# LiliMeng/network_interpretation_imagenet

Measured on AMD Instinct MI355X. Metric: masked-forward-passes/sec (224x224, resnet101), higher is better.
Workload: dtype f16x3 (split-fp16 MFMA, fp32 accumulate); stem conv in fp32 by superposition over superpixels; 1 GPU; resnet101, 512 masks/image x 128 images per GPU (BASELINE configs[2]; x1 GPUs); images_per_gpu=128, masks_per_image=512, forward_batch=2340, num_cus=256, entry=MaskedForwardEngine.score_packed, stem=table, lib_stamp=53ee82e6fdd921c4570974547a85c605b3493926e4b08dbc956d47bbb7fcb210, lib_stamp_matches_tree=True, product_library=True, parallelism=mask-batch shard x1 + one all_gather of scores

## Files before the change

include/mpx.h:

```cpp
#ifndef MPX_H
#define MPX_H

#include <stddef.h>
#include <stdint.h>

#ifdef __cplusplus
extern "C" {
#endif

#define MPX_IMG 224
#define MPX_IMG_PAD 230
#define MPX_NUM_CLASSES 1000

enum {
    MPX_E_ARG = -1,
    MPX_E_STATE = -2,
    MPX_E_NOMEM = -3,
    MPX_E_INTERNAL = -4
};

#define MPX_ARCH_MNIST_NET 1
#define MPX_ARCH_CIFAR_RESNET 2000
#define MPX_ARCH_VGG 3000
#define MPX_ARCH_VGG_BN 3100
#define MPX_ARCH_ALEXNET 4000
#define MPX_ARCH_DENSENET 5000
#define MPX_ARCH_MOBILENET 6000
#define MPX_ARCH_SQUEEZENET 7000
#define MPX_ARCH_GOOGLENET 8000
#define MPX_ARCH_SHUFFLENET 9000
#define MPX_ARCH_EFFICIENTNET 10000
typedef struct mpx_engine mpx_engine;

typedef struct mpx_conv_desc {
    char name[48];
    char bn_name[48];
    int32_t cin, cout, ksize, stride, pad;
    int32_t hin, hout;
    int32_t relu;
    int32_t residual;
    int32_t k_packed;
    int32_t cout_pad;
} mpx_conv_desc;

int mpx_create(int arch_id, int max_batch, int device, mpx_engine** out);
int mpx_destroy(mpx_engine* h);
const char* mpx_last_error(const mpx_engine* h);
int mpx_max_batch(const mpx_engine* h);
int mpx_num_cus(const mpx_engine* h);
int mpx_geometry(const mpx_engine* h, int* image_size, int* in_channels, int* num_classes, int* logit_pitch);
size_t mpx_workspace_bytes(const mpx_engine* h);

int mpx_num_convs(const mpx_engine* h);
int mpx_conv_info(const mpx_engine* h, int i, mpx_conv_desc* out);
int mpx_conv_out_slice(const mpx_engine* h, int i, int* pitch, int* offset);
int mpx_conv_in_slice(const mpx_engine* h, int i, int* pitch, int* offset, int* bf, int* hp);
int mpx_conv_consumer_act(const mpx_engine* h, int i, int* act);

int mpx_set_conv_weights(mpx_engine* h, int i, const float* w, const float* conv_bias, const float* gamma,
                         const float* beta, const float* mean, const float* var, float eps);
int mpx_weights_complete(const mpx_engine* h);

typedef struct mpx_norm_desc {
    char name[64];
    int32_t channels;
    int32_t hw;
} mpx_norm_desc;
int mpx_num_norms(const mpx_engine* h);
int mpx_norm_info(const mpx_engine* h, int k, mpx_norm_desc* out);
int mpx_load_norm(mpx_engine* h, int k, const float* gamma, const float* beta, const float* mean, const float* var, float eps);
int mpx_norm_params(const mpx_engine* h, int k, const float** scale, const float** shift);

typedef struct mpx_dwconv_desc {
    char name[48];
    char bn_name[48];
    int32_t channels;
    int32_t pitch;
    int32_t stride;
    int32_t hin;
    int32_t clamp_in;
} mpx_dwconv_desc;
int mpx_num_dwconvs(const mpx_engine* h);
int mpx_dwconv_info(const mpx_engine* h, int k, mpx_dwconv_desc* out);
int mpx_load_dwconv(mpx_engine* h, int k, const float* w, const float* gamma, const float* beta, const float* mean, const float* var, float eps);
int mpx_dwconv_params(const mpx_engine* h, int k, const float** w, const float** scale, const float** shift);
int mpx_dwconv_layout(const mpx_engine* h, int k, int* linear, int* bf, int* hp);
int mpx_dwconv_shape(const mpx_engine* h, int k, int* ksize, int* act_in, int* act_out);

typedef struct mpx_se_desc {
    char name[48];
    int32_t channels;
    int32_t pitch;
    int32_t q;
    int32_t hw;
} mpx_se_desc;
int mpx_num_se(const mpx_engine* h);
int mpx_se_info(const mpx_engine* h, int k, mpx_se_desc* out);
int mpx_load_se(mpx_engine* h, int k, const float* w1, const float* b1, const float* w2, const float* b2);
int mpx_se_params(const mpx_engine* h, int k, const float** w1, const float** b1, const float** w2, const float** b2);

int mpx_set_conv_tile(mpx_engine* h, int i, int tile);
int mpx_get_conv_tile(const mpx_engine* h, int i);
int mpx_last_conv_kernels(const mpx_engine* h);

int mpx_pack_conv_weights(const mpx_conv_desc* d, const float* w, const float* conv_bias, const float* gamma,
                          const float* beta, const float* mean, const float* var, float eps,
                          uint16_t* w_hi, uint16_t* w_lo, float* scale, float* shift);
int mpx_mask_apply_normalize(mpx_engine* h, const uint8_t* img_u8_hwc, const float* img_f32_chw,
                             const int32_t* seg, const uint8_t* onoff, int M, int S,
                             const float mean[3], const float std[3], int slot0,
                             float* out_f32_nchw, void* stream);

int mpx_stem_table_build(mpx_engine* h, const uint8_t* img_u8_hwc, const float* img_f32_chw, const int32_t* seg, int S,
                         const float mean[3], const float std[3], void* stream);
int mpx_stem_table_apply(mpx_engine* h, const uint8_t* onoff, int M, int S, int slot0, void* stream);

int mpx_mask_apply_minmax(mpx_engine* h, const float* img_f32_chw, const int32_t* seg, const uint8_t* removed,
                          int M, int S, int slot0, float* out_f32_nchw, void* stream);

int mpx_avgpool2_pad(mpx_engine* h, const void* in_hi, const void* in_lo, void* out_hi, void* out_lo, int B,
                     int hin, int cin_p, int cout_p, void* stream);

int mpx_conv_bn_act(mpx_engine* h, int i, const void* in_hi, const void* in_lo,
                    const void* res_hi, const void* res_lo, void* out_hi, void* out_lo,
                    float* out_f32, int B, void* stream);

int mpx_conv_dual_bn_act(mpx_engine* h, int i, const void* in_hi, const void* in_lo, const void* x_hi,
                         const void* x_lo, void* out_hi, void* out_lo, int B, void* stream);
int mpx_set_fusion(mpx_engine* h, int mask);

int mpx_bottleneck_tail(mpx_engine* h, int i, const void* t1_hi, const void* t1_lo, const void* x_hi, const void* x_lo,
                        void* out_hi, void* out_lo, void* next_hi, void* next_lo, int B, void* stream);
int mpx_num_bottleneck_tails(const mpx_engine* h);
int mpx_bottleneck_tail_info(const mpx_engine* h, int k, int* conv2, int* conv3, int* downsample, int* next_conv1);

int mpx_maxpool3x3s2(mpx_engine* h, const void* in_hi, const void* in_lo, void* out_hi,
                     void* out_lo, int B, int hin, int c, void* stream);

int mpx_maxpool2x2s2(mpx_engine* h, const void* in_hi, const void* in_lo, void* out_hi,
                     void* out_lo, int B, int hin, int c, void* stream);

int mpx_maxpool3x3s2p0(mpx_engine* h, const void* in_hi, const void* in_lo, void* out_hi,
                       void* out_lo, int B, int hin, int c, void* stream);

int mpx_maxpool3x3_clip(mpx_engine* h, const void* in_hi, const void* in_lo, void* out_hi, void* out_lo, int B, int hin, int stride, int pad,
                        int pitch, void* stream);
int mpx_num_clip_pools(const mpx_engine* h);
int mpx_clip_pool_info(const mpx_engine* h, int k, int* hin, int* stride, int* pad, int* pitch);

int mpx_concat_bn_relu(mpx_engine* h, const void* fresh_hi, const void* fresh_lo, int g, int fresh_stride, void* raw_hi, void* raw_lo,
                       int c_total, int c_old, const float* scale, const float* shift, void* out_hi, void* out_lo, int c_norm,
                       long long npix, void* stream);

int mpx_avgpool2x2s2(mpx_engine* h, const void* in_hi, const void* in_lo, void* out_hi, void* out_lo, int B, int hin, int c,
                     void* stream);

int mpx_dwconv3x3_bn_relu6(mpx_engine* h, const void* in_hi, const void* in_lo, const float* w, const float* scale, const float* shift,
                           void* out_hi, void* out_lo, int B, int hin, int pitch, int stride, int clamp_in, void* stream);

int mpx_dwconv3x3_bn(mpx_engine* h, const void* in_hi, const void* in_lo, const float* w, const float* scale, const float* shift,
                     void* out_hi, void* out_lo, int B, int hin, int pitch, int stride, void* stream);

int mpx_dwconv_bn_act(mpx_engine* h, const void* in_hi, const void* in_lo, const float* w, const float* scale, const float* shift,
                      void* out_hi, void* out_lo, int B, int hin, int pitch, int ksize, int stride, int act_in, int act_out, void* stream);

int mpx_se_gate(mpx_engine* h, const void* in_hi, const void* in_lo, const float* w1, const float* b1, const float* w2, const float* b2,
                float* gate, int B, int hw, int pitch, int q, void* stream);

int mpx_se_scale(mpx_engine* h, const void* in_hi, const void* in_lo, const float* gate, void* out_hi, void* out_lo, int B, int hw, int pitch,
                 void* stream);

int mpx_shuffle2_concat(mpx_engine* h, const void* a_hi, const void* a_lo, int a_pitch, const void* b_hi, const void* b_lo, int b_pitch,
                        void* out_hi, void* out_lo, int B, int hw, int bf, int hp, void* stream);
int mpx_num_shuffles(const mpx_engine* h);
int mpx_shuffle_info(const mpx_engine* h, int k, int* hw, int* bf, int* hp, int* a_pitch, int* b_pitch);

int mpx_global_avgpool_clamp6(mpx_engine* h, const void* in_hi, const void* in_lo, void* out_hi, void* out_lo, int B, int hw,
                              int c, void* stream);

int mpx_global_avgpool_silu(mpx_engine* h, const void* in_hi, const void* in_lo, void* out_hi, void* out_lo, int B, int hw, int c,
                            void* stream);

int mpx_global_avgpool_logits(mpx_engine* h, const void* in_hi, const void* in_lo, float* out_f32, int B, int hw, int c, int out_pitch,
                              void* stream);

int mpx_stem_conv_maxpool(mpx_engine* h, void* out_hi, void* out_lo, int B, void* stream);

int mpx_global_avgpool(mpx_engine* h, const void* in_hi, const void* in_lo, void* out_hi,
                       void* out_lo, int B, int hw, int c, void* stream);

int mpx_head_softmax_gather(mpx_engine* h, const float* logits, const int32_t* label,
                            float* score, int32_t* pred, int B, void* stream);

int mpx_forward(mpx_engine* h, const int32_t* label, float* score, int32_t* pred,
                float* logits_out, int B, void* stream);

int mpx_heatmap_accumulate(mpx_engine* h, const int32_t* seg, const uint8_t* onoff, const int32_t* pred,
                           const int32_t* label, int M, int S, float* heat, void* stream);

int mpx_input_planes(const mpx_engine* h, void** hi, void** lo);
int mpx_mark_input_staged(mpx_engine* h, int slot0, int M);
int mpx_stem_planes(const mpx_engine* h, void** hi, void** lo);
int mpx_profile_enable(mpx_engine* h, int on);
int mpx_profile_collect(mpx_engine* h, double ms_by_kind[4], long long launches_by_kind[4],
                        double* per_conv_ms);
int mpx_profile_collect_ex(mpx_engine* h, double ms_by_kind[4], long long launches_by_kind[4], double* per_conv_ms,
                           double* per_norm_ms, double* avgpool2_ms);
int mpx_profile_collect_dw(mpx_engine* h, double ms_by_kind[4], long long launches_by_kind[4], double* per_conv_ms,
                           double* per_norm_ms, double* avgpool2_ms, double* per_dw_ms);
int mpx_profile_collect_pool(mpx_engine* h, double ms_by_kind[4], long long launches_by_kind[4], double* per_conv_ms,
                             double* per_norm_ms, double* avgpool2_ms, double* per_dw_ms, double* per_clip_pool_ms);
int mpx_profile_collect_shuffle(mpx_engine* h, double ms_by_kind[4], long long launches_by_kind[4], double* per_conv_ms,
                                double* per_norm_ms, double* avgpool2_ms, double* per_dw_ms, double* per_clip_pool_ms, double* per_shuffle_ms);
int mpx_profile_collect_se(mpx_engine* h, double ms_by_kind[4], long long launches_by_kind[4], double* per_conv_ms, double* per_norm_ms,
                           double* avgpool2_ms, double* per_dw_ms, double* per_clip_pool_ms, double* per_shuffle_ms, double* per_se_gate_ms,
                           double* per_se_scale_ms);
double mpx_flops_per_forward(const mpx_engine* h);

#ifdef __cplusplus
}
#endif
#endif
```

network_interpretation_imagenet_amd/_lib.py:

```python
import ctypes as C
import os

import torch

_HERE = os.path.dirname(os.path.abspath(__file__))
PRODUCT_LIB_PATH = os.path.join(_HERE, "libmpx.so")
LIB_PATH = os.environ.get("MPX_LIB_PATH") or PRODUCT_LIB_PATH

IMG = 224
IMG_PAD = 230
NUM_CLASSES = 1000


class MpxError(RuntimeError):
    pass


class ConvDesc(C.Structure):
    _fields_ = [("name", C.c_char * 48), ("bn_name", C.c_char * 48),
                ("cin", C.c_int32), ("cout", C.c_int32), ("ksize", C.c_int32),
                ("stride", C.c_int32), ("pad", C.c_int32), ("hin", C.c_int32),
                ("hout", C.c_int32), ("relu", C.c_int32), ("residual", C.c_int32),
                ("k_packed", C.c_int32), ("cout_pad", C.c_int32)]


class NormDesc(C.Structure):
    _fields_ = [("name", C.c_char * 64), ("channels", C.c_int32), ("hw", C.c_int32)]


class DwConvDesc(C.Structure):
    _fields_ = [("name", C.c_char * 48), ("bn_name", C.c_char * 48), ("channels", C.c_int32), ("pitch", C.c_int32),
                ("stride", C.c_int32), ("hin", C.c_int32), ("clamp_in", C.c_int32)]


class SeDesc(C.Structure):
    _fields_ = [("name", C.c_char * 48), ("channels", C.c_int32), ("pitch", C.c_int32), ("q", C.c_int32), ("hw", C.c_int32)]


_vp, _i, _f = C.c_void_p, C.c_int, C.c_float
_fp = C.POINTER(C.c_float)

SIGNATURES = {
    "mpx_create": (_i, [_i, _i, _i, C.POINTER(_vp)]),
    "mpx_destroy": (_i, [_vp]),
    "mpx_last_error": (C.c_char_p, [_vp]),
    "mpx_max_batch": (_i, [_vp]),
    "mpx_num_cus": (_i, [_vp]),
    "mpx_workspace_bytes": (C.c_size_t, [_vp]),
    "mpx_num_convs": (_i, [_vp]),
    "mpx_conv_info": (_i, [_vp, _i, C.POINTER(ConvDesc)]),
    "mpx_set_conv_weights": (_i, [_vp, _i, _vp, _vp, _vp, _vp, _vp, _vp, _f]),
    "mpx_geometry": (_i, [_vp, C.POINTER(_i), C.POINTER(_i), C.POINTER(_i), C.POINTER(_i)]),
    "mpx_mask_apply_minmax": (_i, [_vp, _vp, _vp, _vp, _i, _i, _i, _vp, _vp]),
    "mpx_avgpool2_pad": (_i, [_vp, _vp, _vp, _vp, _vp, _i, _i, _i, _i, _vp]),
    "mpx_weights_complete": (_i, [_vp]),
    "mpx_set_conv_tile": (_i, [_vp, _i, _i]),
    "mpx_get_conv_tile": (_i, [_vp, _i]),
    "mpx_last_conv_kernels": (_i, [_vp]),
    "mpx_pack_conv_weights": (_i, [C.POINTER(ConvDesc), _vp, _vp, _vp, _vp, _vp, _vp, _f, _vp, _vp, _vp, _vp]),
    "mpx_mask_apply_normalize": (_i, [_vp, _vp, _vp, _vp, _vp, _i, _i, _fp, _fp, _i, _vp, _vp]),
    "mpx_stem_table_build": (_i, [_vp, _vp, _vp, _vp, _i, _fp, _fp, _vp]),
    "mpx_stem_table_apply": (_i, [_vp, _vp, _i, _i, _i, _vp]),
    "mpx_conv_bn_act": (_i, [_vp, _i, _vp, _vp, _vp, _vp, _vp, _vp, _vp, _i, _vp]),
    "mpx_conv_dual_bn_act": (_i, [_vp, _i, _vp, _vp, _vp, _vp, _vp, _vp, _i, _vp]),
    "mpx_set_fusion": (_i, [_vp, _i]),
    "mpx_bottleneck_tail": (_i, [_vp, _i, _vp, _vp, _vp, _vp, _vp, _vp, _vp, _vp, _i, _vp]),
    "mpx_num_bottleneck_tails": (_i, [_vp]),
    "mpx_bottleneck_tail_info": (_i, [_vp, _i, C.POINTER(_i), C.POINTER(_i), C.POINTER(_i), C.POINTER(_i)]),
    "mpx_stem_conv_maxpool": (_i, [_vp, _vp, _vp, _i, _vp]),
    "mpx_maxpool3x3s2": (_i, [_vp, _vp, _vp, _vp, _vp, _i, _i, _i, _vp]),
    "mpx_maxpool2x2s2": (_i, [_vp, _vp, _vp, _vp, _vp, _i, _i, _i, _vp]),
    "mpx_maxpool3x3s2p0": (_i, [_vp, _vp, _vp, _vp, _vp, _i, _i, _i, _vp]),
    "mpx_global_avgpool": (_i, [_vp, _vp, _vp, _vp, _vp, _i, _i, _i, _vp]),
    "mpx_head_softmax_gather": (_i, [_vp, _vp, _vp, _vp, _vp, _i, _vp]),
    "mpx_forward": (_i, [_vp, _vp, _vp, _vp, _vp, _i, _vp]),
    "mpx_heatmap_accumulate": (_i, [_vp, _vp, _vp, _vp, _vp, _i, _i, _vp, _vp]),
    "mpx_input_planes": (_i, [_vp, C.POINTER(_vp), C.POINTER(_vp)]),
    "mpx_mark_input_staged": (_i, [_vp, _i, _i]),
    "mpx_stem_planes": (_i, [_vp, C.POINTER(_vp), C.POINTER(_vp)]),
    "mpx_profile_enable": (_i, [_vp, _i]),
    "mpx_profile_collect": (_i, [_vp, C.POINTER(C.c_double), C.POINTER(C.c_longlong), C.POINTER(C.c_double)]),
    "mpx_flops_per_forward": (C.c_double, [_vp]),
    "mpx_num_norms": (_i, [_vp]),
    "mpx_norm_info": (_i, [_vp, _i, C.POINTER(NormDesc)]),
    "mpx_load_norm": (_i, [_vp, _i, _vp, _vp, _vp, _vp, _f]),
    "mpx_norm_params": (_i, [_vp, _i, C.POINTER(_vp), C.POINTER(_vp)]),
    "mpx_concat_bn_relu": (_i, [_vp, _vp, _vp, _i, _i, _vp, _vp, _i, _i, _vp, _vp, _vp, _vp, _i, C.c_longlong, _vp]),
    "mpx_avgpool2x2s2": (_i, [_vp, _vp, _vp, _vp, _vp, _i, _i, _i, _vp]),
    "mpx_profile_collect_ex": (_i, [_vp, C.POINTER(C.c_double), C.POINTER(C.c_longlong), C.POINTER(C.c_double), C.POINTER(C.c_double),
                                    C.POINTER(C.c_double)]),
    "mpx_num_dwconvs": (_i, [_vp]),
    "mpx_dwconv_info": (_i, [_vp, _i, C.POINTER(DwConvDesc)]),
    "mpx_load_dwconv": (_i, [_vp, _i, _vp, _vp, _vp, _vp, _vp, _f]),
    "mpx_dwconv_params": (_i, [_vp, _i, C.POINTER(_vp), C.POINTER(_vp), C.POINTER(_vp)]),
    "mpx_dwconv3x3_bn_relu6": (_i, [_vp, _vp, _vp, _vp, _vp, _vp, _vp, _vp, _i, _i, _i, _i, _i, _vp]),
    "mpx_global_avgpool_clamp6": (_i, [_vp, _vp, _vp, _vp, _vp, _i, _i, _i, _vp]),
    "mpx_profile_collect_dw": (_i, [_vp, C.POINTER(C.c_double), C.POINTER(C.c_longlong), C.POINTER(C.c_double), C.POINTER(C.c_double),
                                    C.POINTER(C.c_double), C.POINTER(C.c_double)]),
    "mpx_conv_out_slice": (_i, [_vp, _i, C.POINTER(C.c_int), C.POINTER(C.c_int)]),
    "mpx_global_avgpool_logits": (_i, [_vp, _vp, _vp, _vp, _i, _i, _i, _i, _vp]),
    "mpx_maxpool3x3_clip": (_i, [_vp, _vp, _vp, _vp, _vp, _i, _i, _i, _i, _i, _vp]),
    "mpx_num_clip_pools": (_i, [_vp]),
    "mpx_clip_pool_info": (_i, [_vp, _i, C.POINTER(C.c_int), C.POINTER(C.c_int), C.POINTER(C.c_int), C.POINTER(C.c_int)]),
    "mpx_profile_collect_pool": (_i, [_vp, C.POINTER(C.c_double), C.POINTER(C.c_longlong), C.POINTER(C.c_double), C.POINTER(C.c_double),
                                      C.POINTER(C.c_double), C.POINTER(C.c_double), C.POINTER(C.c_double)]),
    "mpx_dwconv3x3_bn": (_i, [_vp, _vp, _vp, _vp, _vp, _vp, _vp, _vp, _i, _i, _i, _i, _vp]),
    "mpx_dwconv_layout": (_i, [_vp, _i, C.POINTER(C.c_int), C.POINTER(C.c_int), C.POINTER(C.c_int)]),
    "mpx_shuffle2_concat": (_i, [_vp, _vp, _vp, _i, _vp, _vp, _i, _vp, _vp, _i, _i, _i, _i, _vp]),
    "mpx_num_shuffles": (_i, [_vp]),
    "mpx_shuffle_info": (_i, [_vp, _i, C.POINTER(C.c_int), C.POINTER(C.c_int), C.POINTER(C.c_int), C.POINTER(C.c_int), C.POINTER(C.c_int)]),
    "mpx_conv_in_slice": (_i, [_vp, _i, C.POINTER(C.c_int), C.POINTER(C.c_int), C.POINTER(C.c_int), C.POINTER(C.c_int)]),
    "mpx_profile_collect_shuffle": (_i, [_vp, C.POINTER(C.c_double), C.POINTER(C.c_longlong), C.POINTER(C.c_double), C.POINTER(C.c_double),
                                         C.POINTER(C.c_double), C.POINTER(C.c_double), C.POINTER(C.c_double), C.POINTER(C.c_double)]),
    "mpx_conv_consumer_act": (_i, [_vp, _i, C.POINTER(C.c_int)]),
    "mpx_dwconv_shape": (_i, [_vp, _i, C.POINTER(C.c_int), C.POINTER(C.c_int), C.POINTER(C.c_int)]),
    "mpx_dwconv_bn_act": (_i, [_vp, _vp, _vp, _vp, _vp, _vp, _vp, _vp, _i, _i, _i, _i, _i, _i, _i, _vp]),
    "mpx_num_se": (_i, [_vp]),
    "mpx_se_info": (_i, [_vp, _i, C.POINTER(SeDesc)]),
    "mpx_load_se": (_i, [_vp, _i, _vp, _vp, _vp, _vp]),
    "mpx_se_params": (_i, [_vp, _i, C.POINTER(_vp), C.POINTER(_vp), C.POINTER(_vp), C.POINTER(_vp)]),
    "mpx_se_gate": (_i, [_vp, _vp, _vp, _vp, _vp, _vp, _vp, _vp, _i, _i, _i, _i, _vp]),
    "mpx_se_scale": (_i, [_vp, _vp, _vp, _vp, _vp, _vp, _i, _i, _i, _vp]),
    "mpx_global_avgpool_silu": (_i, [_vp, _vp, _vp, _vp, _vp, _i, _i, _i, _vp]),
    "mpx_profile_collect_se": (_i, [_vp, C.POINTER(C.c_double), C.POINTER(C.c_longlong)] + [C.POINTER(C.c_double)] * 8),
}

_lib = None


def load():
    global _lib
    if _lib is None:
        if not os.path.exists(LIB_PATH):
            raise MpxError("HIP extension %s not built; run `python -c 'import __graft_entry__ as g; g.build()'` "
                           "(hipcc --offload-arch=gfx950). There is no CPU fallback." % LIB_PATH)
        if is_probe_build():
            import sys
            sys.stderr.write("mpx: binding %s (MPX_LIB_PATH / with_lib.py) -- NOT the product library %s; probe builds may be timing-only\n"
                             % (LIB_PATH, PRODUCT_LIB_PATH))
        lib = C.CDLL(LIB_PATH)
        for name, (res, args) in SIGNATURES.items():
            fn = getattr(lib, name)
            fn.restype = res
            fn.argtypes = args
        _lib = lib
    return _lib


def is_probe_build():
    return os.path.realpath(LIB_PATH) != os.path.realpath(PRODUCT_LIB_PATH)


def bound_library():
    import hashlib
    h = hashlib.sha256()
    with open(LIB_PATH, "rb") as fh:
        for chunk in iter(lambda: fh.read(1 << 20), b""):
            h.update(chunk)
    stamp = None
    if os.path.exists(LIB_PATH + ".sha256"):
        with open(LIB_PATH + ".sha256") as fh:
            stamp = fh.read().strip()
    return {"lib_path": LIB_PATH, "lib_sha256": h.hexdigest(), "lib_stamp": stamp, "product_library": not is_probe_build()}


def check(handle, rc, what):
    if rc != 0:
        msg = load().mpx_last_error(handle).decode() if handle else ""
        raise MpxError("%s failed (rc=%d): %s" % (what, rc, msg))
```

network_interpretation_imagenet_amd/csrc/mpx_api.hip:

```cpp
#include "../../include/mpx.h"
#include "mpx_kernels.h"
#include "mpx_conv3p.h"
#include "mpx_conv3pp.h"
#include "mpx_conv256.h"
#include "mpx_conv256p.h"
#include "mpx_convx.h"
#include "mpx_convw.h"
#include "mpx_btail.h"
#include "mpx_stemtab.h"
#include "mpx_dw.h"
#include "mpx_fire.h"
#include "mpx_pool3c.h"
#include "mpx_shuffle.h"
#include "mpx_mbconv.h"

#include <algorithm>
#include <cmath>
#include <cstdarg>
#include <initializer_list>
#include <new>
#include <cstdio>
#include <cstdlib>
#include <cstring>
#include <string>
#include <vector>

using namespace mpx;

namespace {

constexpr int kActBufs = 4;
constexpr int kStemK = 7;
constexpr int kProfilePairs = 4096;
constexpr size_t kActElemsPerImage = 112 * 112 * 64;
constexpr size_t kVggActElemsPerImage = 224 * 224 * 64;
constexpr size_t kAlexActElemsPerImage = 55 * 55 * 64;
constexpr size_t kMobileActElemsPerImage = 112 * 112 * 96;
constexpr size_t kSqueezeActElemsPerImage = 111 * 111 * 64;
constexpr size_t kShuffleActElemsPerImage = 112 * 112 * 32;
constexpr size_t kEffActElemsPerImage = 112 * 112 * 96;
constexpr int kSmallCPad = 32;

enum OpKind { OP_CONV = 0, OP_MAXPOOL = 1, OP_AVGPOOL = 2, OP_HEAD = 3, OP_AVGPAD = 4, OP_BTAIL = 5, OP_MAXPOOL2 = 6, OP_MAXPOOL3P0 = 7,
              OP_CATNORM = 8, OP_AVGPOOL2 = 9, OP_DWCONV = 10, OP_AVGPOOL6 = 11, OP_AVGLOGITS = 12, OP_MAXPOOL3C = 13, OP_SHUFFLE = 14,
              OP_SEGATE = 15, OP_SESCALE = 16, OP_AVGPOOLSILU = 17 };
enum Buf { BUF_INPUT = -1, BUF_POOL = -2, BUF_NONE = -3, BUF_STEM = -4 };

struct ConvLayer {
    mpx_conv_desc d;
    half_t* w_hi = nullptr;
    half_t* w_lo = nullptr;
    float* scale = nullptr;
    float* shift = nullptr;
    bool loaded = false;
    bool is_fc = false;
    bool is_stem = false;
    int consumer_act = 0;
    bool has_bias = false;
    int cin_pad = 0;
    int cout_store = 0;
    int y_pitch = 0;
    int y_offset = 0;
    int x_pitch = 0;
    int x_offset = 0;
    int in_bf = 0;
    int in_hp = 0;
    int tile = 0;
    int tile_default = -1;
    int fuse_partner = -1;
    bool fuse_main = false;
    half_t* fw_hi = nullptr;
    half_t* fw_lo = nullptr;
    float* fscale = nullptr;
    float* fshift = nullptr;
    bool fused_loaded = false;
    std::vector<float> hw, hgamma, hbeta, hmean, hvar;
    float heps = 0.f;
};

struct Op {
    int kind;
    int conv;
    int in, out, res;
    int hin, c;
    int in2;
    int z = BUF_NONE;
    int g = 0, ctot = 0;
};

struct NormLayer {
    mpx_norm_desc d;
    float* scale = nullptr;
    float* shift = nullptr;
    bool loaded = false;
};

struct TailBlock {
    int c1 = -1, c2 = -1, c3 = -1, ds = -1, next1 = -1;
    half_t* w3p_hi = nullptr;
    half_t* w3p_lo = nullptr;
    bool ready = false;
};

struct DwLayer {
    mpx_dwconv_desc d;
    bool linear = false;
    int in_bf = 0, in_hp = 0;
    int ksize = 3;
    bool mb = false;
    int act_in = 0, act_out = 0;
    float* w = nullptr;
    float* scale = nullptr;
    float* shift = nullptr;
    bool loaded = false;
};

struct SeLayer {
    mpx_se_desc d;
    float* w1 = nullptr;
    float* b1 = nullptr;
    float* w2 = nullptr;
    float* b2 = nullptr;
    bool loaded = false;
};

constexpr int kProfSubDw = -100;
constexpr int kProfSubPool3c = -1000000;
constexpr int kProfSubShuffle = -2000000;
constexpr int kProfSubSeGate = -3000000;
constexpr int kProfSubSeScale = -4000000;

struct ShuffleOp {
    int side, bf, hp, a_pitch, b_pitch, b_offset;
};

struct ClipPool {
    int hin, stride, pad, pitch;
};

struct ProfRec {
    hipEvent_t t0, t1;
    int kind;
    int conv;
    int sub;
};

}

struct mpx_engine {
    int arch = 0, max_batch = 0, device = 0;
    int num_cus = 256;
    int img = MPX_IMG, in_ch = 3, ncls = MPX_NUM_CLASSES, logit_pitch = MPX_NUM_CLASSES;
    bool small = false;
    bool vgg = false;
    bool alexnet = false;
    bool densenet = false;
    std::vector<NormLayer> norms;
    bool mobilenet = false;
    std::vector<DwLayer> dws;
    bool squeezenet = false;
    bool googlenet = false;
    std::vector<ClipPool> pools3c;
    bool shufflenet = false;
    std::vector<ShuffleOp> shuffles;
    bool efficientnet = false;
    std::vector<SeLayer> ses;
    float* se_gate = nullptr;
    int se_pitch_max = 0;
    int n_act_bufs = kActBufs;
    size_t act_elems_per_image = 0;
    float* k0_scratch = nullptr;
    bool bottleneck = false;
    int feat = 0;
    std::vector<ConvLayer> convs;
    std::vector<Op> ops;
    std::vector<Op> ops_bt;
    std::vector<TailBlock> tails;
    int ops_bt_x = 0;
    bool fuse_bt = true;
    char* arena = nullptr;
    size_t arena_bytes = 0;
    char* tab_arena = nullptr;
    size_t tab_arena_bytes = 0;
    half_t* in_hi = nullptr;
    half_t* in_lo = nullptr;
    half_t* act_hi[kActBufs] = {};
    half_t* act_lo[kActBufs] = {};
    half_t* pool_hi = nullptr;
    half_t* pool_lo = nullptr;
    float* logits = nullptr;
    float* seg_scratch = nullptr;
    half_t* stem_hi = nullptr;
    half_t* stem_lo = nullptr;
    float* stem_w32 = nullptr;
    float* stem_s32 = nullptr;
    float* stem_t32 = nullptr;
    int* tab_cnt = nullptr;
    int* tab_off = nullptr;
    int* tab_lab = nullptr;
    int* tab_heavy = nullptr;
    float* tab_vec = nullptr;
    unsigned* tab_bits = nullptr;
    size_t tab_sizes[4] = {0, 0, 0, 0};
    int tab_S = -1;
    bool stem_w_loaded = false;
    std::vector<uint8_t> slot_src;
    std::string err;
    bool in_forward = false;
    unsigned last_kernels = 0;
    bool fuse_ds = true;
    bool fuse_pool = true;
    bool prof_on = false;
    std::vector<ProfRec> prof_pool;
    int prof_used = 0;
    hipStream_t prof_stream = nullptr;
#ifdef MPX_DIAG
    unsigned long long* stamps = nullptr;
#endif
};

namespace {

int fail(mpx_engine* h, int code, const char* fmt, ...) {
    if (h) {
        char buf[512];
        va_list ap;
        va_start(ap, fmt);
        vsnprintf(buf, sizeof buf, fmt, ap);
        va_end(ap);
        h->err = buf;
    }
    return code;
}

#define MPX_HIP(h, call)                                                                         \
    do {                                                                                         \
        hipError_t e_ = (call);                                                                  \
        if (e_ != hipSuccess)                                                                    \
            return fail((h), (int)e_, "%s failed: %s (%s:%d)", #call, hipGetErrorString(e_),     \
                        __FILE__, __LINE__);                                                     \
    } while (0)

#define MPX_SET_DEVICE(h)                                   \
    do {                                                    \
        if (!(h)->in_forward) MPX_HIP((h), hipSetDevice((h)->device)); \
    } while (0)

size_t round_up(size_t v, size_t a) { return (v + a - 1) / a * a; }

void set_name(char* dst, const std::string& s) {
    std::snprintf(dst, 48, "%s", s.c_str());
}

int default_tile(const mpx_conv_desc& d);
bool patch_eligible(const mpx_conv_desc& d);

int build_topology_small(mpx_engine* h);
int build_topology_vgg(mpx_engine* h);
int build_topology_alexnet(mpx_engine* h);
int build_topology_densenet(mpx_engine* h);
int build_topology_mobilenet(mpx_engine* h);
int build_topology_squeezenet(mpx_engine* h);
int build_topology_googlenet(mpx_engine* h);
int build_topology_shufflenet(mpx_engine* h);
int build_topology_efficientnet(mpx_engine* h);

int build_topology(mpx_engine* h) {
    if (h->arch == MPX_ARCH_MNIST_NET || (h->arch > MPX_ARCH_CIFAR_RESNET && h->arch < MPX_ARCH_CIFAR_RESNET + 1000))
        return build_topology_small(h);
    if (h->arch > MPX_ARCH_VGG && h->arch < MPX_ARCH_VGG_BN + 100) return build_topology_vgg(h);
    if (h->arch >= MPX_ARCH_ALEXNET && h->arch < MPX_ARCH_ALEXNET + 100) return build_topology_alexnet(h);
    if (h->arch >= MPX_ARCH_DENSENET && h->arch < MPX_ARCH_DENSENET + 1000) return build_topology_densenet(h);
    if (h->arch >= MPX_ARCH_MOBILENET && h->arch < MPX_ARCH_MOBILENET + 1000) return build_topology_mobilenet(h);
    if (h->arch >= MPX_ARCH_SQUEEZENET && h->arch < MPX_ARCH_SQUEEZENET + 1000) return build_topology_squeezenet(h);
    if (h->arch >= MPX_ARCH_GOOGLENET && h->arch < MPX_ARCH_GOOGLENET + 1000) return build_topology_googlenet(h);
    if (h->arch >= MPX_ARCH_SHUFFLENET && h->arch < MPX_ARCH_SHUFFLENET + 1000) return build_topology_shufflenet(h);
    if (h->arch >= MPX_ARCH_EFFICIENTNET && h->arch < MPX_ARCH_EFFICIENTNET + 1000) return build_topology_efficientnet(h);
    h->act_elems_per_image = kActElemsPerImage;
    int depths[4];
    switch (h->arch) {
        case 18: depths[0] = 2; depths[1] = 2; depths[2] = 2; depths[3] = 2; h->bottleneck = false; break;
        case 34: depths[0] = 3; depths[1] = 4; depths[2] = 6; depths[3] = 3; h->bottleneck = false; break;
        case 50: depths[0] = 3; depths[1] = 4; depths[2] = 6; depths[3] = 3; h->bottleneck = true; break;
        case 101: depths[0] = 3; depths[1] = 4; depths[2] = 23; depths[3] = 3; h->bottleneck = true; break;
        case 152: depths[0] = 3; depths[1] = 8; depths[2] = 36; depths[3] = 3; h->bottleneck = true; break;
        default: return MPX_E_ARG;
    }
    const int exp = h->bottleneck ? 4 : 1;
    auto add_conv = [&](const std::string& name, const std::string& bn, int cin, int cout, int k, int stride,
                        int pad, int hin, int relu, int residual) {
        ConvLayer L;
        std::memset(&L.d, 0, sizeof L.d);
        set_name(L.d.name, name);
        set_name(L.d.bn_name, bn);
        L.d.cin = cin; L.d.cout = cout; L.d.ksize = k; L.d.stride = stride; L.d.pad = pad;
        L.d.hin = hin; L.d.hout = (hin + 2 * pad - k) / stride + 1;
        L.d.relu = relu; L.d.residual = residual;
        L.is_stem = (cin == 3);
        L.cin_pad = cin;
        L.cout_store = cout;
        L.d.k_packed = L.is_stem ? kStemK * 32 : k * k * cin;
        L.d.cout_pad = (int)round_up(cout, 128);
        L.tile = default_tile(L.d);
        h->convs.push_back(L);
        return (int)h->convs.size() - 1;
    };
    auto add_op = [&](int kind, int conv, int in, int out, int res, int hin, int c, int in2 = BUF_NONE) {
        Op o{kind, conv, in, out, res, hin, c, in2};
        h->ops.push_back(o);
    };
    auto pick = [&](std::initializer_list<int> busy) {
        for (int b = 0; b < kActBufs; ++b) {
            bool used = false;
            for (int u : busy) used |= (u == b);
            if (!used) return b;
        }
        return -100;
    };

    int c = add_conv("conv1", "bn1", 3, 64, 7, 2, 3, 224, 1, 0);
    add_op(OP_CONV, c, BUF_INPUT, 0, BUF_NONE, 0, 0);
    add_op(OP_MAXPOOL, -1, 0, BUF_STEM, BUF_NONE, 112, 64);
    int X = BUF_STEM, cin = 64, hcur = 56;
    const int widths[4] = {64, 128, 256, 512};
    struct BlockRec { int c1, c2, c3, ds, hin; };
    std::vector<BlockRec> blocks;
    for (int s = 0; s < 4; ++s) {
        const int w = widths[s];
        for (int b = 0; b < depths[s]; ++b) {
            const int stride = (b == 0 && s > 0) ? 2 : 1;
            const std::string p = "layer" + std::to_string(s + 1) + "." + std::to_string(b) + ".";
            const bool ds = (b == 0) && (stride != 1 || cin != w * exp);
            const int hout = hcur / stride;
            if (!h->bottleneck) {
                const int T1 = pick({X});
                c = add_conv(p + "conv1", p + "bn1", cin, w, 3, stride, 1, hcur, 1, 0);
                add_op(OP_CONV, c, X, T1, BUF_NONE, 0, 0);
                int res = X, T2 = -100;
                if (ds) {
                    T2 = pick({X, T1});
                    c = add_conv(p + "downsample.0", p + "downsample.1", cin, w * exp, 1, stride, 0, hcur, 0, 0);
                    add_op(OP_CONV, c, X, T2, BUF_NONE, 0, 0);
                    res = T2;
                }
                const int O = pick({X, T1, T2});
                c = add_conv(p + "conv2", p + "bn2", w, w, 3, 1, 1, hout, 1, 1);
                add_op(OP_CONV, c, T1, O, res, 0, 0);
                X = O;
            } else {
                BlockRec R{-1, -1, -1, -1, hcur};
                const int T1 = pick({X});
                R.c1 = c = add_conv(p + "conv1", p + "bn1", cin, w, 1, 1, 0, hcur, 1, 0);
                add_op(OP_CONV, c, X, T1, BUF_NONE, 0, 0);
                const int T2 = pick({X, T1});
                R.c2 = c = add_conv(p + "conv2", p + "bn2", w, w, 3, stride, 1, hcur, 1, 0);
                add_op(OP_CONV, c, T1, T2, BUF_NONE, 0, 0);
                int res = X, dsc = -1;
                if (ds) {
                    const int T3 = pick({X, T1, T2});
                    R.ds = dsc = add_conv(p + "downsample.0", p + "downsample.1", cin, w * exp, 1, stride, 0, hcur, 0, 0);
                    add_op(OP_CONV, dsc, X, T3, BUF_NONE, 0, 0);
                    res = T3;
                }
                R.c3 = c = add_conv(p + "conv3", p + "bn3", w, w * exp, 1, 1, 0, hout, 1, 1);
                add_op(OP_CONV, c, T2, T1, res, 0, 0, ds ? X : BUF_NONE);
                if (ds) {
                    h->convs[c].fuse_partner = dsc; h->convs[c].fuse_main = true;
                    h->convs[dsc].fuse_partner = c;
                }
                blocks.push_back(R);
                X = T1;
            }
            cin = w * exp;
            hcur = hout;
        }
    }
    {
        auto tail_ok = [&](size_t k) {
            if (k + 1 >= blocks.size()) return false;
            const mpx_conv_desc& d2 = h->convs[blocks[k].c2].d;
            const mpx_conv_desc& d3 = h->convs[blocks[k].c3].d;
            const mpx_conv_desc& n1 = h->convs[blocks[k + 1].c1].d;
            if (!(d2.cin == BT_MID && d2.cout == BT_MID && d2.ksize == 3 && d2.stride == 1 && d2.hin == 56)) return false;
            if (!(d3.cin == BT_MID && d3.cout == BT_OUT)) return false;
            if (blocks[k].ds >= 0) {
                const mpx_conv_desc& dd = h->convs[blocks[k].ds].d;
                if (!(dd.cin == BT_MID && dd.stride == 1 && dd.ksize == 1)) return false;
            }
            return n1.cin == BT_OUT && n1.ksize == 1 && n1.stride == 1 && n1.hin == 56 && (n1.cout == 64 || n1.cout == 128) &&
                   !(blocks[k].ds >= 0 && n1.cout != 64);
        };
        bool any = false;
        for (size_t k = 0; k < blocks.size(); ++k) any |= tail_ok(k);
        if (any) {
            std::vector<Op>& out = h->ops_bt;
            out.push_back(h->ops[0]);
            out.push_back(h->ops[1]);
            int Xb = BUF_STEM, T1c = -100;
            for (size_t k = 0; k < blocks.size(); ++k) {
                const BlockRec& R = blocks[k];
                int T1 = T1c;
#ifdef BT_NO_HEAD
                const bool whole = false;
#else
                const bool whole = tail_ok(k) && R.ds >= 0 && T1 < 0;
#endif
                if (T1 < 0 && !whole) {
                    T1 = pick({Xb});
                    out.push_back(Op{OP_CONV, R.c1, Xb, T1, BUF_NONE, 0, 0, BUF_NONE});
                }
                T1c = -100;
                if (tail_ok(k)) {
                    TailBlock tb;
                    tb.c1 = R.c1; tb.c2 = R.c2; tb.c3 = R.c3; tb.ds = R.ds; tb.next1 = blocks[k + 1].c1;
                    h->tails.push_back(tb);
                    if (whole) T1 = BUF_NONE;
                    const int O = pick({Xb, T1}), Z = pick({Xb, T1, O});
                    Op o{OP_BTAIL, (int)h->tails.size() - 1, T1, O, Xb, 0, 0, BUF_NONE};
                    o.z = Z;
                    out.push_back(o);
                    Xb = O;
                    T1c = Z;
                    continue;
                }
                const int T2 = pick({Xb, T1});
                out.push_back(Op{OP_CONV, R.c2, T1, T2, BUF_NONE, 0, 0, BUF_NONE});
                int res = Xb;
                if (R.ds >= 0) {
                    const int T3 = pick({Xb, T1, T2});
                    out.push_back(Op{OP_CONV, R.ds, Xb, T3, BUF_NONE, 0, 0, BUF_NONE});
                    res = T3;
                }
                out.push_back(Op{OP_CONV, R.c3, T2, T1, res, 0, 0, R.ds >= 0 ? Xb : BUF_NONE});
                Xb = T1;
            }
            h->ops_bt_x = Xb;
        }
    }
    h->feat = cin;
    add_op(OP_AVGPOOL, -1, X, BUF_POOL, BUF_NONE, hcur, cin);
    c = add_conv("fc", "", cin, MPX_NUM_CLASSES, 1, 1, 0, 1, 0, 0);
    h->convs[c].is_fc = true;
    add_op(OP_CONV, c, BUF_POOL, BUF_NONE, BUF_NONE, 0, 0);
    add_op(OP_HEAD, -1, BUF_NONE, BUF_NONE, BUF_NONE, 0, 0);
    if (!h->ops_bt.empty()) {
        h->ops_bt.push_back(Op{OP_AVGPOOL, -1, h->ops_bt_x, BUF_POOL, BUF_NONE, hcur, cin, BUF_NONE});
        h->ops_bt.push_back(h->ops[h->ops.size() - 2]);
        h->ops_bt.push_back(h->ops[h->ops.size() - 1]);
    }
    return 0;
}

int build_topology_small(mpx_engine* h) {
    h->small = true;
    h->ncls = 10;
    h->logit_pitch = 16;
    auto add_conv = [&](const std::string& name, const std::string& bn, int cin, int cout, int k, int stride, int pad,
                        int hin, int relu, int residual, bool bias, bool fc) {
        ConvLayer L;
        std::memset(&L.d, 0, sizeof L.d);
        set_name(L.d.name, name);
        set_name(L.d.bn_name, bn);
        L.d.cin = cin; L.d.cout = cout; L.d.ksize = k; L.d.stride = stride; L.d.pad = pad;
        L.d.hin = hin; L.d.hout = (hin + 2 * pad - k) / stride + 1;
        L.d.relu = relu; L.d.residual = residual;
        L.has_bias = bias;
        L.is_fc = fc;
        L.cin_pad = (int)round_up(cin, kSmallCPad);
        L.cout_store = fc ? h->logit_pitch : (int)round_up(cout, kSmallCPad);
        L.d.k_packed = k * k * L.cin_pad;
        L.d.cout_pad = (int)round_up(cout, 128);
        L.tile = default_tile(L.d);
        h->convs.push_back(L);
        return (int)h->convs.size() - 1;
    };
    auto add_op = [&](int kind, int conv, int in, int out, int res, int hin, int c) {
        Op o{kind, conv, in, out, res, hin, c, BUF_NONE};
        h->ops.push_back(o);
    };
    int feat = 0, hlast = 0, X = 0;
    size_t act = 0;
    auto track = [&](int hout, int c) { act = std::max(act, (size_t)hout * hout * round_up(c, kSmallCPad)); };
    if (h->arch == MPX_ARCH_MNIST_NET) {
        h->img = 28; h->in_ch = 1;
        const int cfg[5][3] = {{1, 32, 1}, {32, 32, 1}, {32, 64, 2}, {64, 64, 1}, {64, 128, 2}};
        int hcur = 28, in = BUF_INPUT;
        for (int i = 0; i < 5; ++i) {
            const std::string n = "conv" + std::to_string(i + 1);
            const int c = add_conv(n + ".0", n + ".1", cfg[i][0], cfg[i][1], 3, cfg[i][2], 1, hcur, 1, 0, true, false);
            const int out = (in == 0) ? 1 : 0;
            add_op(OP_CONV, c, in, out, BUF_NONE, 0, 0);
            in = out;
            hcur = h->convs[c].d.hout;
            track(hcur, cfg[i][1]);
        }
        const int c6 = add_conv("conv6", "", 128, 128, 3, 1, 1, hcur, 0, 0, true, false);
        X = (in == 0) ? 1 : 0;
        add_op(OP_CONV, c6, in, X, BUF_NONE, 0, 0);
        feat = 128; hlast = hcur;
        h->feat = feat;
        add_op(OP_AVGPOOL, -1, X, BUF_POOL, BUF_NONE, hlast, feat);
        const int cf = add_conv("fc1", "", feat, 10, 1, 1, 0, 1, 0, 0, true, true);
        add_op(OP_CONV, cf, BUF_POOL, BUF_NONE, BUF_NONE, 0, 0);
    } else {
        const int depth = h->arch - MPX_ARCH_CIFAR_RESNET;
        if (depth < 8 || (depth - 2) % 6 != 0) return MPX_E_ARG;
        const int n = (depth - 2) / 6;
        h->img = 32; h->in_ch = 3;
        int c = add_conv("conv1", "bn1", 3, 16, 3, 1, 1, 32, 1, 0, false, false);
        add_op(OP_CONV, c, BUF_INPUT, 0, BUF_NONE, 0, 0);
        track(32, 16);
        X = 0;
        int inplanes = 16, hcur = 32;
        const int planes_of[3] = {16, 32, 64};
        for (int sidx = 0; sidx < 3; ++sidx) {
            const int planes = planes_of[sidx];
            for (int b = 0; b < n; ++b) {
                const int stride = (sidx > 0 && b == 0) ? 2 : 1;
                const std::string p = "layer" + std::to_string(sidx + 1) + "." + std::to_string(b) + ".";
                int busy[3] = {X, -1, -1};
                auto pick = [&]() {
                    for (int q = 0; q < kActBufs; ++q)
                        if (q != busy[0] && q != busy[1] && q != busy[2]) return q;
                    return -100;
                };
                const int T1 = pick();
                busy[1] = T1;
                c = add_conv(p + "conv1", p + "bn1", inplanes, planes, 3, stride, 1, hcur, 1, 0, false, false);
                add_op(OP_CONV, c, X, T1, BUF_NONE, 0, 0);
                const int hout = h->convs[c].d.hout;
                int res = X;
                if (stride != 1 || inplanes != planes) {
                    const int T2 = pick();
                    busy[2] = T2;
                    add_op(OP_AVGPAD, -1, X, T2, BUF_NONE, hcur, (int)round_up(inplanes, kSmallCPad) * 65536 + (int)round_up(planes, kSmallCPad));
                    res = T2;
                }
                const int O = pick();
                c = add_conv(p + "conv2", p + "bn2", planes, planes, 3, 1, 1, hout, 1, 1, false, false);
                add_op(OP_CONV, c, T1, O, res, 0, 0);
                X = O;
                inplanes = planes;
                hcur = hout;
                track(hcur, planes);
            }
        }
        feat = 64; hlast = hcur;
        h->feat = feat;
        add_op(OP_AVGPOOL, -1, X, BUF_POOL, BUF_NONE, hlast, feat);
        const int cf = add_conv("fc", "", feat, 10, 1, 1, 0, 1, 0, 0, true, true);
        add_op(OP_CONV, cf, BUF_POOL, BUF_NONE, BUF_NONE, 0, 0);
    }
    add_op(OP_HEAD, -1, BUF_NONE, BUF_NONE, BUF_NONE, 0, 0);
    h->act_elems_per_image = act;
    return 0;
}

int build_topology_vgg(mpx_engine* h) {
    const bool bn = h->arch > MPX_ARCH_VGG_BN;
    const int depth = h->arch - (bn ? MPX_ARCH_VGG_BN : MPX_ARCH_VGG);
    constexpr int M = 0;
    static const int cfg_a[] = {64, M, 128, M, 256, 256, M, 512, 512, M, 512, 512, M};
    static const int cfg_b[] = {64, 64, M, 128, 128, M, 256, 256, M, 512, 512, M, 512, 512, M};
    static const int cfg_d[] = {64, 64, M, 128, 128, M, 256, 256, 256, M, 512, 512, 512, M, 512, 512, 512, M};
    static const int cfg_e[] = {64, 64, M, 128, 128, M, 256, 256, 256, 256, M, 512, 512, 512, 512, M, 512, 512, 512, 512, M};
    const int* cfg = nullptr;
    int n = 0;
    switch (depth) {
        case 11: cfg = cfg_a; n = (int)(sizeof cfg_a / sizeof *cfg_a); break;
        case 13: cfg = cfg_b; n = (int)(sizeof cfg_b / sizeof *cfg_b); break;
        case 16: cfg = cfg_d; n = (int)(sizeof cfg_d / sizeof *cfg_d); break;
        case 19: cfg = cfg_e; n = (int)(sizeof cfg_e / sizeof *cfg_e); break;
        default: return MPX_E_ARG;
    }
    h->vgg = true;
    h->n_act_bufs = 2;
    h->act_elems_per_image = kVggActElemsPerImage;
    auto add_conv = [&](const std::string& name, const std::string& bn_name, int cin, int cout, int k, int pad, int hin, int relu, bool fc) {
        ConvLayer L;
        std::memset(&L.d, 0, sizeof L.d);
        set_name(L.d.name, name);
        set_name(L.d.bn_name, bn_name);
        L.d.cin = cin; L.d.cout = cout; L.d.ksize = k; L.d.stride = 1; L.d.pad = pad;
        L.d.hin = hin; L.d.hout = hin + 2 * pad - k + 1;
        L.d.relu = relu;
        L.has_bias = true;
        L.is_fc = fc;
        L.is_stem = (cin == 3);
        L.cin_pad = cin;
        L.cout_store = cout;
        L.d.k_packed = L.is_stem ? k * 32 : k * k * cin;
        L.d.cout_pad = (int)round_up(cout, 128);
        L.tile = default_tile(L.d);
        h->convs.push_back(L);
        return (int)h->convs.size() - 1;
    };
    auto add_op = [&](int kind, int conv, int in, int out, int hin, int c) {
        h->ops.push_back(Op{kind, conv, in, out, BUF_NONE, hin, c, BUF_NONE});
    };
    int X = BUF_INPUT, cin = 3, hcur = MPX_IMG, idx = 0;
    for (int j = 0; j < n; ++j) {
// ... 701 lines not shown
        return launched(h, id);
    }
    if constexpr (DUAL) {
        if (p.k1) {
            if (((p.k1 >> 5) - Cfg::NSX) < 0 || (((p.k1 >> 5) - Cfg::NSX) & 1))
                return fail(h, MPX_E_INTERNAL, "dual conv: k1/32 - ring depth must be even and >= 0");
            hipLaunchKernelGGL((conv_f16x3_kernel<Cfg, true>), dim3((unsigned)tiles), dim3(Cfg::NT), Cfg::LDS, st, p);
            return launched(h, id);
        }
    }
    hipLaunchKernelGGL((conv_f16x3_kernel<Cfg>), dim3((unsigned)tiles), dim3(Cfg::NT), Cfg::LDS, st, p);
    return launched(h, id);
}

int launch_conv256(mpx_engine* h, int id, const ConvLayer& L, ConvParams& p, hipStream_t st) {
    long long tiles;
    if (int rc = conv_tiles(h, p, L.d.cout_pad, Conv256::TC, Conv256::TP, tiles)) return rc;
    hipLaunchKernelGGL(conv256_f16x3_kernel, dim3((unsigned)tiles), dim3(Conv256::NT), Conv256::LDS, st, p);
    return launched(h, id);
}

int launch_conv256p(mpx_engine* h, int id, const ConvLayer& L, ConvParams& p, hipStream_t st) {
    if (p.r_hi) return launch_tile(h, 9, L, p, st);
    long long tiles;
    if (int rc = conv_tiles(h, p, L.d.cout_pad, Conv256P::TC, Conv256P::TP, tiles)) return rc;
    const long long grid = persistent_grid(h, p, tiles);
    if (grid <= 0 || tiles < h->num_cus) return launch_tile(h, 2, L, p, st);
    hipLaunchKernelGGL(conv256p_f16x3_kernel<false>, dim3((unsigned)grid), dim3(Conv256P::NT), Conv256P::LDS, st, p);
    return launched(h, id);
}

bool conv256p_dual_eligible(const ConvLayer& L, const ConvLayer& D) {
    return !L.is_fc && !L.is_stem && L.cin_pad == L.d.cin && D.cin_pad == D.d.cin && conv256_eligible(L.d) && D.d.ksize == 1 && D.d.pad == 0 &&
           D.d.cin % 64 == 0;
}

int launch_conv256p_dual(mpx_engine* h, const ConvLayer& L, ConvParams& p, hipStream_t st) {
    if (p.k1 <= 0 || p.k1 % 64 != 0 || (p.ktot - p.k1) <= 0 || (p.ktot - p.k1) % 64 != 0 || p.r_hi)
        return fail(h, MPX_E_INTERNAL, "dual 256x256 conv: k1 = %d and k2 = %d must be multiples of 64, without a residual operand", p.k1, p.ktot - p.k1);
    long long tiles;
    if (int rc = conv_tiles(h, p, L.d.cout_pad, Conv256P::TC, Conv256P::TP, tiles)) return rc;
    const long long grid = persistent_grid(h, p, tiles);
    if (grid <= 0 || tiles < h->num_cus) return 0;
    hipLaunchKernelGGL(conv256p_f16x3_kernel<true>, dim3((unsigned)grid), dim3(Conv256P::NT), Conv256P::LDS, st, p);
    if (int rc = launched(h, 13)) return rc;
    return 1;
}

int launch_convx(mpx_engine* h, int id, const ConvLayer& L, ConvParams& p, hipStream_t st) {
    long long tiles;
    if (int rc = conv_tiles(h, p, L.d.cout_pad, ConvX::TC, ConvX::TP, tiles)) return rc;
    const long long grid = persistent_grid(h, p, tiles);
    if (grid <= 0 || tiles < h->num_cus) return launch_tile(h, 7, L, p, st);
    hipLaunchKernelGGL(convx_f16x3_kernel, dim3((unsigned)grid), dim3(ConvX::NT), ConvX::LDS, st, p);
    return launched(h, id);
}

int launch_convw(mpx_engine* h, int id, const ConvLayer& L, ConvParams& p, hipStream_t st) {
    if (p.ktot != ConvW::K) return fail(h, MPX_E_INTERNAL, "convw: K = %d (the kernel holds K = %d in registers)", p.ktot, ConvW::K);
    if (!p.relu || !p.r_hi) return launch_tile(h, 10, L, p, st);
    long long tiles;
    if (int rc = conv_tiles(h, p, L.d.cout_pad, ConvW::TC, ConvW::TP, tiles)) return rc;
    const long long grid = persistent_grid(h, p, tiles);
    if (grid <= 0 || tiles < 2LL * h->num_cus) return launch_tile(h, 7, L, p, st);
    hipLaunchKernelGGL((convw_f16x3_kernel<ConvW::K, true>), dim3((unsigned)grid), dim3(ConvW::NT), ConvW::LDS, st, p);
    return launched(h, id);
}

template <class PC>
int launch_conv_patch(mpx_engine* h, int id, const ConvLayer& L, ConvParams& p, hipStream_t st) {
    long long tiles;
    if (int rc = conv_tiles(h, p, L.d.cout_pad, PC::TC, PC::TP, tiles)) return rc;
    p.patch_rows = patch_rows_needed(L.d.hin, PC::TP);
    hipLaunchKernelGGL(conv3x3p_f16x3_kernel<PC>, dim3((unsigned)tiles), dim3(PC::NT), PC::lds_bytes(p.patch_rows), st, p);
    return launched(h, id);
}

template <class PC>
int launch_conv_patchp(mpx_engine* h, int id, const ConvLayer& L, ConvParams& p, hipStream_t st) {
    long long tiles;
    if (int rc = conv_tiles(h, p, L.d.cout_pad, PC::TC, PC::TP, tiles)) return rc;
    const long long grid = persistent_grid(h, p, tiles);
    const int H = L.d.hin;
    const long long padded = (long long)(p.M / (H * H) + 2) * (H + 2) * (H + 2);
    if (grid <= 0 || tiles < h->num_cus || p.r_hi || padded >= (1 << 23)) return launch_conv_patch<PC>(h, 6, L, p, st);
    p.patch_rows = patch_rows_needed(H, PC::TP);
    hipLaunchKernelGGL(conv3x3pp_f16x3_kernel<PC>, dim3((unsigned)grid), dim3(PC::NT), PatchPersistent<PC>::lds_bytes(p.patch_rows), st, p);
    return launched(h, id);
}

int launch_patch(mpx_engine* h, int id, const ConvLayer& L, ConvParams& p, hipStream_t st) {
    if (L.d.cout <= 64) return launch_conv_patch<PatchTile1>(h, id, L, p, st);
    return patch_fits<PatchTile0>(L.d) ? launch_conv_patch<PatchTile0>(h, id, L, p, st) : launch_conv_patch<PatchTile2>(h, id, L, p, st);
}

int launch_patchp(mpx_engine* h, int id, const ConvLayer& L, ConvParams& p, hipStream_t st) {
    return patchp_fits<PatchTile0>(L.d) ? launch_conv_patchp<PatchTile0>(h, id, L, p, st) : launch_conv_patchp<PatchTile2>(h, id, L, p, st);
}

struct TileRow {
    int id;
    LaunchFn launch;
    bool (*eligible)(const mpx_conv_desc&);
    const char* refusal;
    int dual;
    bool split;
};

const TileRow kTiles[] = {
    {0, launch_conv_tile<ConvTile0>, nullptr, nullptr, -1, false},
    {1, launch_conv_tile<ConvTile1>, nullptr, nullptr, -1, false},
    {2, launch_conv_tile<ConvTile2, true>, nullptr, nullptr, 2, false},
    {4, launch_conv_tile<ConvTile4>, nullptr, nullptr, -1, false},
    {6, launch_patch, patch_eligible, "the patch kernel needs a 3x3 stride-1 layer whose input patch fits the LDS", -1, false},
    {7, launch_conv_tile<ConvTile7, true>, nullptr, nullptr, 7, false},
    {9, launch_conv256, conv256_eligible, "the 256x256 kernel runs 1x1 stride-1 layers with cout % 256 == 0 and cin % 64 == 0", -1, true},
    {10, launch_convx, convx_eligible,
     "the persistent expanding-1x1 kernel runs 1x1 stride-1 layers with cout % 256 == 0 and cin % 64 == 0, cin >= 128", 7, false},
    {12, launch_patchp, patchp_eligible,
     "the persistent patch kernel needs a 3x3 stride-1 layer with cout >= 128 and no residual operand whose input patch fits the LDS", -1, false},
    {13, launch_conv256p, conv256p_eligible,
     "the persistent 256x256 kernel runs 1x1 stride-1 layers with cout % 256 == 0, cin % 64 == 0 and no residual operand", -1, true},
    {14, launch_convw, convw_eligible,
     "the weights-in-registers expanding-1x1 kernel runs 1x1 stride-1 layers with cout % 256 == 0 and cin = 256", 7, false},
};

struct KernelLds {
    const void* kernel;
    int bytes;
};
const KernelLds kKernelLds[] = {
    {(const void*)conv_f16x3_kernel<ConvTile0>, ConvTile0::LDS},
    {(const void*)conv_f16x3_kernel<ConvTile1>, ConvTile1::LDS},
    {(const void*)conv_f16x3_kernel<ConvTile1, false, true>, ConvTile1::LDS},
    {(const void*)conv_f16x3_kernel<ConvTile2>, ConvTile2::LDS},
    {(const void*)conv_f16x3_kernel<ConvTile7>, ConvTile7::LDS},
    {(const void*)conv_f16x3_kernel<ConvTile2, true>, ConvTile2::LDS},
    {(const void*)conv_f16x3_kernel<ConvTile7, true>, ConvTile7::LDS},
    {(const void*)conv256_f16x3_kernel, Conv256::LDS},
    {(const void*)convx_f16x3_kernel, ConvX::LDS},
    {(const void*)convw_f16x3_kernel<ConvW::K, true>, ConvW::LDS},
    {(const void*)conv256p_f16x3_kernel<false>, Conv256P::LDS},
    {(const void*)conv256p_f16x3_kernel<true>, Conv256P::LDS},
    {(const void*)conv_f16x3_kernel<ConvTile4>, ConvTile4::LDS},
    {(const void*)conv_f16x3_kernel<ConvTile0, false, false, true>, ConvTile0::LDS},
    {(const void*)conv_f16x3_kernel<ConvTile1, false, false, true>, ConvTile1::LDS},
    {(const void*)conv_f16x3_kernel<ConvTile2, false, false, true>, ConvTile2::LDS},
    {(const void*)conv_f16x3_kernel<ConvTile4, false, false, true>, ConvTile4::LDS},
    {(const void*)conv_f16x3_kernel<ConvTile7, false, false, true>, ConvTile7::LDS},
    {(const void*)btail_f16x3_kernel<BtResC64>, BtResC64::LDS},
    {(const void*)btail_f16x3_kernel<BtResC128>, BtResC128::LDS},
    {(const void*)btail_f16x3_kernel<BtDualC64>, BtDualC64::LDS},
    {(const void*)btail_f16x3_kernel<BtHeadC64>, BtHeadC64::LDS},
    {(const void*)conv3x3p_f16x3_kernel<PatchTile0>, kLdsLimit},
    {(const void*)conv3x3p_f16x3_kernel<PatchTile1>, kLdsLimit},
    {(const void*)conv3x3p_f16x3_kernel<PatchTile2>, kLdsLimit},
    {(const void*)conv3x3pp_f16x3_kernel<PatchTile0>, kLdsLimit},
    {(const void*)conv3x3pp_f16x3_kernel<PatchTile2>, kLdsLimit},
};

const TileRow* find_tile(int id) {
    for (const TileRow& r : kTiles)
        if (r.id == id) return &r;
    return nullptr;
}

bool eligible(const TileRow& r, const ConvLayer& L) {
    return !r.eligible || (!L.is_fc && !L.is_stem && L.cin_pad == L.d.cin && !L.y_pitch && !L.x_pitch && r.eligible(L.d));
}

int launch_tile(mpx_engine* h, int id, const ConvLayer& L, ConvParams& p, hipStream_t st) {
    const TileRow* r = find_tile(id);
    if (!r) return fail(h, MPX_E_INTERNAL, "conv: no kernel for tile id %d", id);
    return r->launch(h, id, L, p, st);
}

int default_tile(const mpx_conv_desc& d) {
    if (d.cout <= 64) return d.ksize >= 3 ? 1 : 4;
#ifndef MPX_PROBE_NO_PERSISTENT_PATCH
    if (patchp_eligible(d) && (d.hout >= 14 || (d.hout == 13 && ((d.cout / 128) & (d.cout / 128 - 1)) == 0))) return 12;
#endif
    if (patch_eligible(d)) return 6;
    if (d.ksize == 3) return 0;
    if (d.ksize == 5 && d.cout % 128 != 0 && d.cout % 64 == 0) return 1;
    if (d.ksize == 6) return 2;
#ifndef MPX_PROBE_NO_CONVW
    if (convw_eligible(d) && d.cout > d.cin && d.hout >= 14) return 14;
#endif
    if (convx_eligible(d) && d.cout > d.cin) return 10;
    if (d.stride == 1 && d.cout > d.cin) return 7;
#ifdef MPX_PROBE_NO_PERSISTENT_256
    if (conv256_eligible(d)) return 9;
#endif
    if (conv256_eligible(d)) return conv256p_eligible(d) ? 13 : 9;
    return 2;
}

int conv_params(mpx_engine* h, const ConvLayer& L, const half_t* in_hi, const half_t* in_lo, half_t* y_hi, half_t* y_lo, int B, ConvParams& p) {
    std::memset(&p, 0, sizeof p);
    p.w_hi = L.w_hi; p.w_lo = L.w_lo; p.scale = L.scale; p.shift = L.shift;
    p.y_hi = y_hi; p.y_lo = y_lo;
    p.cout = L.cout_store;
    p.relu = L.d.relu;
    p.ktot = L.d.k_packed;
    if (L.is_stem) {
        p.x_hi = h->in_hi; p.x_lo = h->in_lo;
        p.hin = MPX_IMG_PAD; p.win = MPX_IMG_PAD; p.pix_stride = 4;
        p.kh = L.d.ksize; p.kw = 1; p.stride = L.d.stride; p.pad = L.d.pad - (MPX_IMG_PAD - MPX_IMG) / 2; p.k_per_tap = L.d.k_packed / L.d.ksize;
    } else {
        p.x_hi = in_hi ? in_hi + L.x_offset : in_hi; p.x_lo = in_lo ? in_lo + L.x_offset : in_lo;
        p.hin = L.d.hin; p.win = L.d.hin; p.pix_stride = L.x_pitch ? L.x_pitch : L.cin_pad;
        p.kh = L.d.ksize; p.kw = L.d.ksize; p.stride = L.d.stride; p.pad = L.d.pad; p.k_per_tap = L.cin_pad;
    }
    p.ho = L.d.hout; p.wo = L.d.hout;
    const long long M = (long long)B * p.ho * p.wo;
    if (M > 0x7fffffffLL) return fail(h, MPX_E_ARG, "batch too large for 32-bit pixel indices");
    p.M = (int)M;
#ifdef MPX_DIAG
    p.stamps = h->stamps;
#endif
    return 0;
}

int launch_conv(mpx_engine* h, int i, const half_t* in_hi, const half_t* in_lo, const half_t* r_hi,
                const half_t* r_lo, half_t* y_hi, half_t* y_lo, float* y_f32, int B, hipStream_t st) {
    const ConvLayer& L = h->convs[i];
    if (!L.loaded) return fail(h, MPX_E_STATE, "layer %d (%s) has no weights", i, L.d.name);
    ConvParams p;
    if (int rc = conv_params(h, L, in_hi, in_lo, y_hi, y_lo, B, p)) return rc;
    if ((long long)B * p.hin * p.win > 0x7fffffffLL) return fail(h, MPX_E_ARG, "batch too large for 32-bit pixel indices");
    p.r_hi = r_hi; p.r_lo = r_lo; p.y_f32 = y_f32;
    if (L.y_pitch) {
        if (r_hi || r_lo || y_f32) return fail(h, MPX_E_ARG, "conv: %s writes a channel slice; it takes no residual operand and no fp32 output", L.d.name);
        p.y_pitch = L.y_pitch;
        p.y_hi += L.y_offset; p.y_lo += L.y_offset;
    }
    ProfScope ps(h, st, OP_CONV, i);
    h->last_kernels = 0;
    const TileRow* row = find_tile(L.tile);
    if (row && row->split && !L.is_stem && !L.y_pitch) {
        const long long M = p.M, tiles_c = (p.cout + Conv256::TC - 1) / Conv256::TC, tiles_p = (M + Conv256::TP - 1) / Conv256::TP;
        const long long total = tiles_p * tiles_c, rounds = total / h->num_cus, rest = total - rounds * h->num_cus;
        const long long howo = (long long)p.ho * p.wo;
        const long long n_a = rounds * h->num_cus / tiles_c * Conv256::TP / howo;
        if (rounds >= 1 && rest > 0 && 2 * rest <= h->num_cus && n_a >= 1 && n_a < B) {
            ConvParams q = p;
            p.M = (int)(n_a * howo);
            int rc = launch_tile(h, L.tile, L, p, st);
            if (rc) return rc;
            const size_t xo = (size_t)n_a * p.hin * p.win * p.pix_stride, yo = (size_t)n_a * howo * p.cout;
            q.M = (int)(M - n_a * howo);
            q.x_hi += xo; q.x_lo += xo;
            q.y_hi += yo; q.y_lo += yo;
            if (q.r_hi) { q.r_hi += yo; q.r_lo += yo; }
            return launch_tile(h, 2, L, q, st);
        }
    }
    return launch_tile(h, L.tile, L, p, st);
}

int launch_conv_fused(mpx_engine* h, int i, const half_t* in_hi, const half_t* in_lo, const half_t* x2_hi,
                      const half_t* x2_lo, half_t* y_hi, half_t* y_lo, int B, hipStream_t st) {
    const ConvLayer& L = h->convs[i];
    if (!L.fuse_main || !L.fused_loaded) return fail(h, MPX_E_STATE, "layer %d (%s) has no fused weights", i, L.d.name);
    const ConvLayer& D = h->convs[L.fuse_partner];
    ConvParams p;
    if (int rc = conv_params(h, L, in_hi, in_lo, y_hi, y_lo, B, p)) return rc;
    if ((long long)B * D.d.hin * D.d.hin > 0x7fffffffLL) return fail(h, MPX_E_ARG, "batch too large for 32-bit pixel indices");
    p.w_hi = L.fw_hi; p.w_lo = L.fw_lo; p.scale = L.fscale; p.shift = L.fshift;
    p.k1 = L.d.cin; p.ktot = L.d.cin + D.d.cin;
    p.x2_hi = x2_hi; p.x2_lo = x2_lo;
    p.hin2 = D.d.hin; p.win2 = D.d.hin; p.pix_stride2 = D.d.cin; p.stride2 = D.d.stride;
    ProfScope ps(h, st, OP_CONV, i);
    h->last_kernels = 0;
    const TileRow* row = find_tile(L.tile);
#ifndef MPX_PROBE_NO_DUAL256P
    if ((L.tile == 9 || L.tile == 10 || L.tile == 13 || L.tile == 14) && conv256p_dual_eligible(L, D)) {
        const int rc = launch_conv256p_dual(h, L, p, st);
        if (rc != 0) return rc < 0 ? rc : 0;
    }
#endif
    return launch_tile(h, row && row->dual >= 0 ? row->dual : 7, L, p, st);
}

bool stem_pool_eligible(const mpx_engine* h) {
    if (h->small || h->googlenet || h->convs.empty()) return false;
    const ConvLayer& L = h->convs[0];
    return L.is_stem && L.d.cout == 64 && L.d.hout == 112 && (L.d.hout / 2) % POOL_PY == 0 && (L.d.hout / 2) % POOL_PX == 0 && L.d.relu;
}

int launch_stem_pool(mpx_engine* h, half_t* y_hi, half_t* y_lo, int B, hipStream_t st) {
    const ConvLayer& L = h->convs[0];
    if (!stem_pool_eligible(h)) return fail(h, MPX_E_STATE, "stem + max pool: this architecture has no 7x7 stem with a max pool");
    if (!L.loaded) return fail(h, MPX_E_STATE, "layer 0 (%s) has no weights", L.d.name);
    ConvParams p;
    if (int rc = conv_params(h, L, nullptr, nullptr, y_hi, y_lo, B, p)) return rc;
    p.n_tiles_c = 1;
    const long long nblocks = (long long)B * (p.ho / 2 / POOL_PY) * (p.wo / 2 / POOL_PX);
    if (nblocks > 0x7fffffffLL) return fail(h, MPX_E_ARG, "conv grid out of range");
    ProfScope ps(h, st, OP_CONV, 0);
    hipLaunchKernelGGL((conv_f16x3_kernel<ConvTile1, false, true>), dim3((unsigned)nblocks), dim3(ConvTile1::NT), ConvTile1::LDS, st, p);
    MPX_HIP(h, hipGetLastError());
    return 0;
}

constexpr int bt_perm_channel(int kpos) {
    const int s = kpos >> 5, q = kpos & 31, g = q >> 3, j = q & 7;
    return 32 * s + (j >> 2) * 16 + 4 * g + (j & 3);
}
constexpr bool bt_perm_is_bijection() {
    bool seen[BT_MID] = {};
    for (int k = 0; k < BT_MID; ++k) {
        const int c = bt_perm_channel(k);
        if (c < 0 || c >= BT_MID || seen[c] || (c >> 5) != (k >> 5)) return false;
        seen[c] = true;
    }
    return true;
}
static_assert(bt_perm_is_bijection(), "K permutation of the block tail's conv3 operand");
static_assert(bt_perm_channel(0) == 0 && bt_perm_channel(3) == 3 && bt_perm_channel(4) == 16 && bt_perm_channel(8) == 4 && bt_perm_channel(36) == 48,
              "K position 8g + j <-> channel (j>>2)*16 + 4g + (j&3): registers 4g..4g+3 of two stacked 16-row accumulator fragments");

int upload_tail_planes(mpx_engine* h, TailBlock& tb, const std::vector<uint16_t>& hi, const std::vector<uint16_t>& lo, int K) {
    std::vector<uint16_t> ph((size_t)BT_OUT * K), pl((size_t)BT_OUT * K);
    for (int row = 0; row < BT_OUT; ++row)
        for (int k = 0; k < K; ++k) {
            const int src = k < BT_MID ? bt_perm_channel(k) : k;
            ph[w_packed_index(row, k, K)] = hi[w_packed_index(row, src, K)];
            pl[w_packed_index(row, k, K)] = lo[w_packed_index(row, src, K)];
        }
    MPX_HIP(h, hipMemcpy(tb.w3p_hi, ph.data(), ph.size() * 2, hipMemcpyHostToDevice));
    MPX_HIP(h, hipMemcpy(tb.w3p_lo, pl.data(), pl.size() * 2, hipMemcpyHostToDevice));
    tb.ready = true;
    return 0;
}

TailBlock* tail_of_conv3(mpx_engine* h, int c3) {
    for (TailBlock& tb : h->tails)
        if (tb.c3 == c3) return &tb;
    return nullptr;
}

bool tails_ready(const mpx_engine* h) {
    if (h->tails.empty()) return false;
    for (const TailBlock& tb : h->tails)
        if (!tb.ready || !h->convs[tb.c2].loaded || !h->convs[tb.next1].loaded || !h->convs[tb.c1].loaded) return false;
    return true;
}

int launch_btail(mpx_engine* h, int ti, const half_t* t_hi, const half_t* t_lo, const half_t* x_hi, const half_t* x_lo,
                 half_t* y_hi, half_t* y_lo, half_t* z_hi, half_t* z_lo, int B, hipStream_t st) {
    const TailBlock& tb = h->tails[ti];
    const ConvLayer& L2 = h->convs[tb.c2];
    const ConvLayer& L3 = h->convs[tb.c3];
    const ConvLayer& N1 = h->convs[tb.next1];
    if (!tb.ready || !L2.loaded || !N1.loaded) return fail(h, MPX_E_STATE, "block tail %s: weights missing", L2.d.name);
    const bool dual = tb.ds >= 0;
    const bool head = t_hi == nullptr;
    if (head && !dual) return fail(h, MPX_E_ARG, "block tail %s: only a block with a downsample branch (64-channel input) can run its own conv1 in the launch", L2.d.name);
    BtParams p;
    std::memset(&p, 0, sizeof p);
    p.t_hi = head ? x_hi : t_hi; p.t_lo = head ? x_lo : t_lo;
    if (head) {
        const ConvLayer& L1 = h->convs[tb.c1];
        if (!L1.loaded) return fail(h, MPX_E_STATE, "block tail %s: weights of %s missing", L2.d.name, L1.d.name);
        if (!(L1.d.cin == BT_MID && L1.d.cout == BT_MID && L1.d.ksize == 1 && L1.d.stride == 1)) return fail(h, MPX_E_INTERNAL, "block tail: %s is not a 64 -> 64 1x1 conv", L1.d.name);
        p.w0_hi = L1.w_hi; p.w0_lo = L1.w_lo; p.sc0 = L1.scale; p.sh0 = L1.shift;
    }
    p.w2_hi = L2.w_hi; p.w2_lo = L2.w_lo; p.sc2 = L2.scale; p.sh2 = L2.shift;
    p.w3_hi = tb.w3p_hi; p.w3_lo = tb.w3p_lo;
    p.sc3 = dual ? L3.fscale : L3.scale; p.sh3 = dual ? L3.fshift : L3.shift;
    p.r_hi = x_hi; p.r_lo = x_lo; p.y_hi = y_hi; p.y_lo = y_lo;
    p.w1_hi = N1.w_hi; p.w1_lo = N1.w_lo; p.sc1 = N1.scale; p.sh1 = N1.shift;
    p.z_hi = z_hi; p.z_lo = z_lo;
    p.B = B; p.H = L2.d.hin; p.W = L2.d.hin;
    if (p.H % BT_TY || p.W % BT_TX) return fail(h, MPX_E_INTERNAL, "block tail: %dx%d map is not a whole number of 8x14 tiles", p.H, p.W);
    p.tiles_x = p.W / BT_TX;
    p.tiles_per_img = (p.H / BT_TY) * p.tiles_x;
    const long long n_tiles = (long long)B * p.tiles_per_img;
    if (n_tiles <= 0 || n_tiles > 0x7fffffffLL) return fail(h, MPX_E_ARG, "block tail: batch out of range");
    p.n_tiles = (int)n_tiles;
#ifdef MPX_DIAG
    p.stamps = h->stamps;
#endif
    const long long resident = 2LL * h->num_cus;
    const unsigned grid = (unsigned)std::min<long long>(resident / 8 * 8, (n_tiles + 7) / 8 * 8);
    ProfScope ps(h, st, OP_CONV, tb.c2);
    if (head) hipLaunchKernelGGL(btail_f16x3_kernel<BtHeadC64>, dim3(grid), dim3(256), BtHeadC64::LDS, st, p);
    else if (dual) hipLaunchKernelGGL(btail_f16x3_kernel<BtDualC64>, dim3(grid), dim3(256), BtDualC64::LDS, st, p);
    else if (N1.d.cout == 128) hipLaunchKernelGGL(btail_f16x3_kernel<BtResC128>, dim3(grid), dim3(256), BtResC128::LDS, st, p);
    else hipLaunchKernelGGL(btail_f16x3_kernel<BtResC64>, dim3(grid), dim3(256), BtResC64::LDS, st, p);
    MPX_HIP(h, hipGetLastError());
    return 0;
}

int build_fused(mpx_engine* h, int main) {
    ConvLayer& L = h->convs[main];
    ConvLayer& D = h->convs[L.fuse_partner];
    const int cout = L.d.cout, k1 = L.d.cin, k2 = D.d.cin, K = k1 + k2, rows = L.d.cout_pad;
    std::vector<uint16_t> hi((size_t)rows * K, 0), lo((size_t)rows * K, 0);
    std::vector<float> sc(rows, 0.f), sh(rows, 0.f), row(K);
    for (int co = 0; co < cout; ++co) {
        const double s3 = (double)L.hgamma[co] / std::sqrt((double)L.hvar[co] + (double)L.heps);
        const double sd = (double)D.hgamma[co] / std::sqrt((double)D.hvar[co] + (double)D.heps);
        double s = std::fmax(std::fabs(s3), std::fabs(sd));
        if (!(s > 0.0) || !std::isfinite(s)) s = 1.0;
        const double r3 = s3 / s, rd = sd / s;
        float mx = 0.f;
        for (int k = 0; k < k1; ++k) { row[k] = (float)((double)L.hw[(size_t)co * k1 + k] * r3); mx = std::fmax(mx, std::fabs(row[k])); }
        for (int k = 0; k < k2; ++k) { row[k1 + k] = (float)((double)D.hw[(size_t)co * k2 + k] * rd); mx = std::fmax(mx, std::fabs(row[k1 + k])); }
        int e = 0;
        if (mx > 0.f && std::isfinite(mx)) {
            int ex;
            std::frexp(mx, &ex);
            e = 10 - ex;
        }
        for (int k = 0; k < K; ++k) {
            const float sv = std::ldexp(row[k], e);
            const half_t vh = (half_t)sv;
            const half_t vl = (half_t)(sv - (float)vh);
            hi[w_packed_index(co, k, K)] = half_bits(vh);
            lo[w_packed_index(co, k, K)] = half_bits(vl);
        }
        sc[co] = (float)std::ldexp(s, -e);
        sh[co] = (float)(((double)L.hbeta[co] - (double)L.hmean[co] * s3) + ((double)D.hbeta[co] - (double)D.hmean[co] * sd));
    }
    MPX_HIP(h, hipMemcpy(L.fw_hi, hi.data(), hi.size() * 2, hipMemcpyHostToDevice));
    MPX_HIP(h, hipMemcpy(L.fw_lo, lo.data(), lo.size() * 2, hipMemcpyHostToDevice));
    MPX_HIP(h, hipMemcpy(L.fscale, sc.data(), sc.size() * 4, hipMemcpyHostToDevice));
    MPX_HIP(h, hipMemcpy(L.fshift, sh.data(), sh.size() * 4, hipMemcpyHostToDevice));
    L.fused_loaded = true;
    if (TailBlock* tb = tail_of_conv3(h, main)) return upload_tail_planes(h, *tb, hi, lo, K);
    return 0;
}

int launch_catnorm(mpx_engine* h, const CatNormParams& p, int norm, hipStream_t st) {
    ProfScope ps(h, st, 2, -1, norm);
    const unsigned long long units = (unsigned long long)p.npix * (unsigned)((p.c_end - p.c_begin) / 8);
    const unsigned grid = (unsigned)std::min<unsigned long long>((units + 255) / 256, (unsigned long long)h->num_cus * 8);
    hipLaunchKernelGGL(concat_bn_relu_kernel, dim3(grid), dim3(256), 0, st, p);
    MPX_HIP(h, hipGetLastError());
    return 0;
}

int launch_dwconv(mpx_engine* h, const DwParams& p, int dw, hipStream_t st, bool linear = false) {
    ProfScope ps(h, st, 2, -1, dw >= 0 ? kProfSubDw - dw : -1);
    if (linear) {
        const int W = p.stride == 1 ? DwRun<1>::W : DwRun<2>::W;
        const unsigned long long units = (unsigned long long)(p.npix / p.ho) * (unsigned)((p.ho + W - 1) / W) * (unsigned)(p.pitch / 8);
        const unsigned grid = (unsigned)std::min<unsigned long long>((units + 255) / 256, (unsigned long long)h->num_cus * (p.stride == 1 ? 8 : 2));
        if (p.stride == 1)
            hipLaunchKernelGGL(dwconv3x3_bn_kernel<1>, dim3(grid), dim3(256), 0, st, p);
        else
            hipLaunchKernelGGL(dwconv3x3_bn_kernel<2>, dim3(grid), dim3(256), 0, st, p);
        MPX_HIP(h, hipGetLastError());
        return 0;
    }
    const unsigned long long units = (unsigned long long)p.npix * (unsigned)(p.pitch / 8);
    const unsigned grid = (unsigned)std::min<unsigned long long>((units + 255) / 256, (unsigned long long)h->num_cus * 8);
    hipLaunchKernelGGL(dwconv3x3_bn_relu6_kernel, dim3(grid), dim3(256), 0, st, p);
    MPX_HIP(h, hipGetLastError());
    return 0;
}

int launch_mbdw(mpx_engine* h, const MbDwParams& p, int ksize, int stride, int dw, hipStream_t st) {
    ProfScope ps(h, st, 2, -1, dw >= 0 ? kProfSubDw - dw : -1);
    const int W = stride == 1 ? 4 : 2;
    const unsigned long long units = (unsigned long long)p.rows * (unsigned)((p.ho + W - 1) / W) * (unsigned)(p.pitch / 8);
    const unsigned grid = (unsigned)std::min<unsigned long long>((units + 255) / 256, (unsigned long long)h->num_cus * (stride == 1 ? 8 : 2));
    if (ksize == 3 && stride == 1) hipLaunchKernelGGL((dwconv_bn_act_kernel<3, 1>), dim3(grid), dim3(256), 0, st, p);
    else if (ksize == 3) hipLaunchKernelGGL((dwconv_bn_act_kernel<3, 2>), dim3(grid), dim3(256), 0, st, p);
    else if (stride == 1) hipLaunchKernelGGL((dwconv_bn_act_kernel<5, 1>), dim3(grid), dim3(256), 0, st, p);
    else hipLaunchKernelGGL((dwconv_bn_act_kernel<5, 2>), dim3(grid), dim3(256), 0, st, p);
    MPX_HIP(h, hipGetLastError());
    return 0;
}

size_t se_gate_lds(int pitch, int q) { return ((size_t)se_gate_slices(pitch) * pitch + pitch + q) * sizeof(float); }

int launch_se_gate(mpx_engine* h, const SeGateParams& p, int B, int k, hipStream_t st) {
    ProfScope ps(h, st, 2, -1, k >= 0 ? kProfSubSeGate - k : -1);
    hipLaunchKernelGGL(se_gate_kernel, dim3((unsigned)B), dim3(256), se_gate_lds(p.pitch, p.q), st, p);
    MPX_HIP(h, hipGetLastError());
    return 0;
}

int launch_se_scale(mpx_engine* h, const SeScaleParams& p, int k, hipStream_t st) {
    ProfScope ps(h, st, 2, -1, k >= 0 ? kProfSubSeScale - k : -1);
    const unsigned grid = (unsigned)std::min<long long>((p.units + 255) / 256, (long long)h->num_cus * 8);
    hipLaunchKernelGGL(se_scale_kernel, dim3(grid), dim3(256), 0, st, p);
    MPX_HIP(h, hipGetLastError());
    return 0;
}

int launch_shuffle(mpx_engine* h, const ShuffleParams& p, int k, hipStream_t st) {
    ProfScope ps(h, st, 2, -1, k >= 0 ? kProfSubShuffle - k : -1);
    const unsigned long long units = (unsigned long long)p.npix * (unsigned)(2 * p.hp / 8);
    const unsigned grid = (unsigned)std::min<unsigned long long>((units + 255) / 256, (unsigned long long)h->num_cus * 8);
    if (p.bf % 8 == 0)
        hipLaunchKernelGGL(shuffle2_concat_kernel<true>, dim3(grid), dim3(256), 0, st, p);
    else
        hipLaunchKernelGGL(shuffle2_concat_kernel<false>, dim3(grid), dim3(256), 0, st, p);
    MPX_HIP(h, hipGetLastError());
    return 0;
}

int launch_pool3c(mpx_engine* h, const half_t* in_hi, const half_t* in_lo, half_t* out_hi, half_t* out_lo, int B, int hin, int stride, int pad,
                  int pitch, int k, hipStream_t st) {
    Pool3cParams p;
    std::memset(&p, 0, sizeof p);
    p.x_hi = in_hi; p.x_lo = in_lo; p.y_hi = out_hi; p.y_lo = out_lo;
    p.hin = hin; p.ho = pool3c_out_side(hin, stride, pad); p.pitch = pitch; p.pad = pad;
    p.runs = (p.ho + (stride == 1 ? Pool3c<1>::W : Pool3c<2>::W) - 1) / (stride == 1 ? Pool3c<1>::W : Pool3c<2>::W);
    p.units = (long long)B * p.ho * p.runs * (pitch / 8);
    ProfScope ps(h, st, 2, -1, k >= 0 ? kProfSubPool3c - k : -1);
    const unsigned grid = (unsigned)std::min<long long>((p.units + 255) / 256, (long long)h->num_cus * 2);
    if (stride == 1)
        hipLaunchKernelGGL(maxpool3x3_clip_kernel<1>, dim3(grid), dim3(256), 0, st, p);
    else
        hipLaunchKernelGGL(maxpool3x3_clip_kernel<2>, dim3(grid), dim3(256), 0, st, p);
    MPX_HIP(h, hipGetLastError());
    return 0;
}

int pack_conv_weights(const mpx_conv_desc* d, int in_bf, int in_hp, const float* w, const float* conv_bias, const float* gamma,
                      const float* beta, const float* mean, const float* var, float eps, uint16_t* w_hi, uint16_t* w_lo, float* scale,
                      float* shift);

}

extern "C" {

int mpx_pack_conv_weights(const mpx_conv_desc* d, const float* w, const float* conv_bias, const float* gamma,
                          const float* beta, const float* mean, const float* var, float eps, uint16_t* w_hi,
                          uint16_t* w_lo, float* scale, float* shift) {
    return pack_conv_weights(d, 0, 0, w, conv_bias, gamma, beta, mean, var, eps, w_hi, w_lo, scale, shift);
}

}

namespace {

int pack_conv_weights(const mpx_conv_desc* d, int in_bf, int in_hp, const float* w, const float* conv_bias, const float* gamma,
                      const float* beta, const float* mean, const float* var, float eps, uint16_t* w_hi, uint16_t* w_lo, float* scale,
                      float* shift) {
    if (!d || !w || !w_hi || !w_lo || !scale || !shift) return MPX_E_ARG;
// ... 845 lines not shown
    hipStream_t st = as_stream(stream);
    ProfScope ps(h, st, 2, -1);
    const int total = B * (c / 8);
    hipLaunchKernelGGL(global_avgpool_silu_kernel, dim3((total + 255) / 256), dim3(256), 0, st, (const half_t*)in_hi, (const half_t*)in_lo,
                       (half_t*)out_hi, (half_t*)out_lo, B, hw, c);
    MPX_HIP(h, hipGetLastError());
    return 0;
}

int mpx_shuffle2_concat(mpx_engine* h, const void* a_hi, const void* a_lo, int a_pitch, const void* b_hi, const void* b_lo, int b_pitch,
                        void* out_hi, void* out_lo, int B, int hw, int bf, int hp, void* stream) {
    if (!h) return MPX_E_ARG;
    auto misaligned = [](const void* q) { return ((uintptr_t)q & 15) != 0; };
    if (!a_hi || !a_lo || !b_hi || !b_lo || !out_hi || !out_lo) return fail(h, MPX_E_ARG, "shuffle2_concat: null pointer");
    if (B <= 0 || hw <= 0 || bf <= 0 || (bf & 1) || hp < bf || (hp & 31) || a_pitch < bf || (a_pitch & 7) || b_pitch < bf || (b_pitch & 7))
        return fail(h, MPX_E_ARG, "shuffle2_concat: B > 0, hw > 0, bf even and > 0, hp >= bf a multiple of 32, pitches >= bf and multiples of 8");
    if (misaligned(a_hi) || misaligned(a_lo) || misaligned(b_hi) || misaligned(b_lo) || misaligned(out_hi) || misaligned(out_lo))
        return fail(h, MPX_E_ARG, "shuffle2_concat: every pointer must be 16-byte aligned");
    ShuffleParams p;
    std::memset(&p, 0, sizeof p);
    p.a_hi = (const half_t*)a_hi; p.a_lo = (const half_t*)a_lo; p.b_hi = (const half_t*)b_hi; p.b_lo = (const half_t*)b_lo;
    p.y_hi = (half_t*)out_hi; p.y_lo = (half_t*)out_lo;
    p.npix = (long long)B * hw * hw;
    p.a_pitch = a_pitch; p.b_pitch = b_pitch; p.bf = bf; p.hp = hp;
    MPX_SET_DEVICE(h);
    return launch_shuffle(h, p, -1, as_stream(stream));
}

int mpx_num_shuffles(const mpx_engine* h) { return h ? (int)h->shuffles.size() : MPX_E_ARG; }

int mpx_shuffle_info(const mpx_engine* h, int k, int* hw, int* bf, int* hp, int* a_pitch, int* b_pitch) {
    if (!h || k < 0 || k >= (int)h->shuffles.size()) return MPX_E_ARG;
    const ShuffleOp& S = h->shuffles[k];
    if (hw) *hw = S.side;
    if (bf) *bf = S.bf;
    if (hp) *hp = S.hp;
    if (a_pitch) *a_pitch = S.a_pitch;
    if (b_pitch) *b_pitch = S.b_pitch;
    return 0;
}

int mpx_conv_in_slice(const mpx_engine* h, int i, int* pitch, int* offset, int* bf, int* hp) {
    if (!h || i < 0 || i >= (int)h->convs.size()) return MPX_E_ARG;
    const ConvLayer& L = h->convs[i];
    if (pitch) *pitch = L.is_stem ? 4 : (L.x_pitch ? L.x_pitch : L.cin_pad);
    if (offset) *offset = L.x_offset;
    if (bf) *bf = L.in_bf;
    if (hp) *hp = L.in_hp;
    return 0;
}

int mpx_global_avgpool_clamp6(mpx_engine* h, const void* in_hi, const void* in_lo, void* out_hi, void* out_lo, int B, int hw,
                              int c, void* stream) {
    if (!h) return MPX_E_ARG;
    if (!in_hi || !in_lo || !out_hi || !out_lo || B <= 0 || hw <= 0 || c <= 0 || (c & 7) || (long long)B * (c / 8) > 0x7fffffffLL)
        return fail(h, MPX_E_ARG, "global_avgpool_clamp6: bad arguments (c multiple of 8)");
    MPX_SET_DEVICE(h);
    hipStream_t st = as_stream(stream);
    ProfScope ps(h, st, 2, -1);
    const int total = B * (c / 8);
    hipLaunchKernelGGL(global_avgpool_clamp6_kernel, dim3((total + 255) / 256), dim3(256), 0, st, (const half_t*)in_hi,
                       (const half_t*)in_lo, (half_t*)out_hi, (half_t*)out_lo, B, hw, c);
    MPX_HIP(h, hipGetLastError());
    return 0;
}

int mpx_global_avgpool_logits(mpx_engine* h, const void* in_hi, const void* in_lo, float* out_f32, int B, int hw, int c, int out_pitch,
                              void* stream) {
    if (!h) return MPX_E_ARG;
    if (!in_hi || !in_lo || !out_f32 || B <= 0 || hw <= 0 || c <= 0 || (c & 7) || out_pitch < c || (long long)B * (c / 8) > 0x7fffffffLL)
        return fail(h, MPX_E_ARG, "global_avgpool_logits: bad arguments (c a multiple of 8, out_pitch >= c)");
    if (((uintptr_t)in_hi | (uintptr_t)in_lo) & 15) return fail(h, MPX_E_ARG, "global_avgpool_logits: the planes must be 16-byte aligned");
    MPX_SET_DEVICE(h);
    hipStream_t st = as_stream(stream);
    ProfScope ps(h, st, 2, -1);
    const int total = B * (c / 8);
    hipLaunchKernelGGL(global_avgpool_logits_kernel, dim3((total + 255) / 256), dim3(256), 0, st, (const half_t*)in_hi,
                       (const half_t*)in_lo, out_f32, B, hw, c, out_pitch);
    MPX_HIP(h, hipGetLastError());
    return 0;
}

int mpx_conv_out_slice(const mpx_engine* h, int i, int* pitch, int* offset) {
    if (!h || !pitch || !offset || i < 0 || i >= (int)h->convs.size()) return MPX_E_ARG;
    const ConvLayer& L = h->convs[i];
    *pitch = L.y_pitch ? L.y_pitch : L.cout_store;
    *offset = L.y_pitch ? L.y_offset : 0;
    return 0;
}

int mpx_avgpool2x2s2(mpx_engine* h, const void* in_hi, const void* in_lo, void* out_hi, void* out_lo, int B, int hin, int c,
                     void* stream) {
    if (!h) return MPX_E_ARG;
    if (!in_hi || !in_lo || !out_hi || !out_lo || B <= 0 || hin <= 0 || (hin & 1) || c <= 0 || (c & 7))
        return fail(h, MPX_E_ARG, "avgpool2x2s2: bad arguments (hin even and > 0, c a positive multiple of 8)");
    if (((uintptr_t)in_hi | (uintptr_t)in_lo | (uintptr_t)out_hi | (uintptr_t)out_lo) & 15)
        return fail(h, MPX_E_ARG, "avgpool2x2s2: the planes must be 16-byte aligned");
    MPX_SET_DEVICE(h);
    hipStream_t st = as_stream(stream);
    ProfScope ps(h, st, 2, -1, -2);
    const size_t total = (size_t)B * (hin / 2) * (hin / 2) * (c / 8);
    const unsigned grid = (unsigned)std::min<size_t>((total + 255) / 256, (size_t)h->num_cus * 8);
    hipLaunchKernelGGL(avgpool2x2s2_kernel, dim3(grid), dim3(256), 0, st, (const half_t*)in_hi, (const half_t*)in_lo,
                       (half_t*)out_hi, (half_t*)out_lo, B, hin, c);
    MPX_HIP(h, hipGetLastError());
    return 0;
}

int mpx_head_softmax_gather(mpx_engine* h, const float* logits, const int32_t* label, float* score, int32_t* pred,
                            int B, void* stream) {
    if (!h) return MPX_E_ARG;
    if (!logits || !label || !score || !pred || B <= 0) return fail(h, MPX_E_ARG, "head_softmax_gather: null pointer or empty batch");
    MPX_SET_DEVICE(h);
    hipStream_t st = as_stream(stream);
    ProfScope ps(h, st, 3, -1);
    hipLaunchKernelGGL(head_softmax_gather_kernel, dim3((B + 3) / 4), dim3(256), 0, st, logits, label, score, pred, B,
                       h->ncls, h->logit_pitch);
    MPX_HIP(h, hipGetLastError());
    return 0;
}

int mpx_forward(mpx_engine* h, const int32_t* label, float* score, int32_t* pred, float* logits_out, int B,
                void* stream) {
    if (!h) return MPX_E_ARG;
    if (!label || !score || !pred || B <= 0) return fail(h, MPX_E_ARG, "forward: null pointer or empty batch");
    if (B > h->max_batch) return fail(h, MPX_E_STATE, "forward: B=%d exceeds max_batch=%d", B, h->max_batch);
    if (mpx_weights_complete(h) != 1) return fail(h, MPX_E_STATE, "forward: weights not loaded for every layer");
    float* logits = logits_out ? logits_out : h->logits;
    MPX_HIP(h, hipSetDevice(h->device));
    struct InForward {
        mpx_engine* e;
        explicit InForward(mpx_engine* e_) : e(e_) { e->in_forward = true; }
        ~InForward() { e->in_forward = false; }
    } scope(h);
    auto hi = [&](int b) -> half_t* { return b == BUF_POOL ? h->pool_hi : (b == BUF_STEM ? h->stem_hi : (b >= 0 ? h->act_hi[b] : nullptr)); };
    auto lo = [&](int b) -> half_t* { return b == BUF_POOL ? h->pool_lo : (b == BUF_STEM ? h->stem_lo : (b >= 0 ? h->act_lo[b] : nullptr)); };
    int rc = 0;
    bool skip_pool = false;
    bool stem_done = false;
    {
        int n_tab = 0, n_k0 = 0;
        for (int i = 0; i < B; ++i) {
            n_tab += h->slot_src[i] == 2;
            n_k0 += h->slot_src[i] == 1;
        }
        if (n_tab && n_tab != B)
            return fail(h, MPX_E_STATE, "forward: %d of the %d slots were staged by mpx_stem_table_apply and %d by mpx_mask_apply_normalize; one forward takes one kind", n_tab, B, n_k0);
        stem_done = n_tab == B;
    }
    bool use_bt = h->fuse_bt && h->fuse_ds && tails_ready(h);
    for (const TailBlock& tb : h->tails)
        for (int li : {tb.c1, tb.c2, tb.c3, tb.next1})
            use_bt = use_bt && h->convs[li].tile == default_tile(h->convs[li].d);
    const std::vector<Op>& ops = use_bt ? h->ops_bt : h->ops;
    for (size_t oi = 0; oi < ops.size(); ++oi) {
        const Op& o = ops[oi];
        if (stem_done && ((o.kind == OP_CONV && o.conv == 0) || (o.kind == OP_MAXPOOL && o.out == BUF_STEM))) continue;
        switch (o.kind) {
            case OP_BTAIL:
                rc = launch_btail(h, o.conv, hi(o.in), lo(o.in), hi(o.res), lo(o.res), hi(o.out), lo(o.out), hi(o.z), lo(o.z), B, as_stream(stream));
                break;
            case OP_CONV:
                if (h->fuse_pool && o.conv == 0 && oi + 1 < ops.size() && ops[oi + 1].kind == OP_MAXPOOL && stem_pool_eligible(h) &&
                    h->convs[0].tile == 1) {
                    const Op& pool = ops[oi + 1];
                    rc = launch_stem_pool(h, hi(pool.out), lo(pool.out), B, as_stream(stream));
                    skip_pool = true;
                    break;
                }
                if (h->fuse_ds && h->convs[o.conv].fuse_partner >= 0) {
                    const ConvLayer& CL = h->convs[o.conv];
                    const ConvLayer& MAIN = CL.fuse_main ? CL : h->convs[CL.fuse_partner];
                    const TileRow* r = find_tile(MAIN.tile);
                    if (MAIN.fused_loaded && r && r->dual >= 0) {
                        if (!CL.fuse_main) break;
                        rc = launch_conv_fused(h, o.conv, hi(o.in), lo(o.in), hi(o.in2), lo(o.in2), hi(o.out), lo(o.out), B, as_stream(stream));
                        break;
                    }
                }
                if (h->convs[o.conv].is_fc)
                    rc = mpx_conv_bn_act(h, o.conv, hi(o.in), lo(o.in), nullptr, nullptr, nullptr, nullptr, logits, B, stream);
                else
                    rc = mpx_conv_bn_act(h, o.conv, hi(o.in), lo(o.in), hi(o.res), lo(o.res), hi(o.out), lo(o.out), nullptr, B, stream);
                break;
            case OP_MAXPOOL:
                if (skip_pool) { skip_pool = false; break; }
                rc = mpx_maxpool3x3s2(h, hi(o.in), lo(o.in), hi(o.out), lo(o.out), B, o.hin, o.c, stream);
                break;
            case OP_MAXPOOL2: rc = mpx_maxpool2x2s2(h, hi(o.in), lo(o.in), hi(o.out), lo(o.out), B, o.hin, o.c, stream); break;
            case OP_MAXPOOL3P0: rc = mpx_maxpool3x3s2p0(h, hi(o.in), lo(o.in), hi(o.out), lo(o.out), B, o.hin, o.c, stream); break;
            case OP_AVGPOOL: rc = mpx_global_avgpool(h, hi(o.in), lo(o.in), hi(o.out), lo(o.out), B, o.hin * o.hin, o.c, stream); break;
            case OP_HEAD: rc = mpx_head_softmax_gather(h, logits, label, score, pred, B, stream); break;
            case OP_AVGPAD: rc = mpx_avgpool2_pad(h, hi(o.in), lo(o.in), hi(o.out), lo(o.out), B, o.hin, o.c >> 16, o.c & 0xffff, stream); break;
            case OP_AVGPOOL2: rc = mpx_avgpool2x2s2(h, hi(o.in), lo(o.in), hi(o.out), lo(o.out), B, o.hin, o.c, stream); break;
            case OP_AVGPOOL6: rc = mpx_global_avgpool_clamp6(h, hi(o.in), lo(o.in), hi(o.out), lo(o.out), B, o.hin * o.hin, o.c, stream); break;
            case OP_AVGLOGITS: rc = mpx_global_avgpool_logits(h, hi(o.in), lo(o.in), logits, B, o.hin * o.hin, o.c, h->logit_pitch, stream); break;
            case OP_MAXPOOL3C: {
                const ClipPool& P = h->pools3c[o.conv];
                rc = launch_pool3c(h, hi(o.in), lo(o.in), hi(o.out), lo(o.out), B, P.hin, P.stride, P.pad, P.pitch, o.conv, as_stream(stream));
                break;
            }
            case OP_DWCONV: {
                const DwLayer& D = h->dws[o.conv];
                if (D.mb) {
                    MbDwParams q;
                    std::memset(&q, 0, sizeof q);
                    q.x_hi = hi(o.in); q.x_lo = lo(o.in); q.y_hi = hi(o.out); q.y_lo = lo(o.out);
                    q.w = D.w; q.scale = D.scale; q.shift = D.shift;
                    q.hin = D.d.hin; q.ho = (D.d.hin - 1) / D.d.stride + 1; q.pitch = D.d.pitch; q.act_in = D.act_in; q.act_out = D.act_out;
                    q.rows = (long long)B * q.ho;
                    rc = launch_mbdw(h, q, D.ksize, D.d.stride, o.conv, as_stream(stream));
                    break;
                }
                DwParams p;
                std::memset(&p, 0, sizeof p);
                p.x_hi = hi(o.in); p.x_lo = lo(o.in); p.y_hi = hi(o.out); p.y_lo = lo(o.out);
                p.w = D.w; p.scale = D.scale; p.shift = D.shift;
                p.hin = D.d.hin; p.ho = (D.d.hin - 1) / D.d.stride + 1; p.pitch = D.d.pitch; p.stride = D.d.stride; p.clamp_in = D.d.clamp_in;
                p.npix = (long long)B * p.ho * p.ho;
                rc = launch_dwconv(h, p, o.conv, as_stream(stream), D.linear);
                break;
            }
            case OP_SEGATE: {
                const SeLayer& E = h->ses[o.conv];
                SeGateParams p;
                std::memset(&p, 0, sizeof p);
                p.x_hi = hi(o.in); p.x_lo = lo(o.in);
                p.w1 = E.w1; p.b1 = E.b1; p.w2 = E.w2; p.b2 = E.b2; p.gate = h->se_gate;
                p.hw = E.d.hw * E.d.hw; p.pitch = E.d.pitch; p.q = E.d.q;
                rc = launch_se_gate(h, p, B, o.conv, as_stream(stream));
                break;
            }
            case OP_SESCALE: {
                const SeLayer& E = h->ses[o.conv];
                SeScaleParams p;
                std::memset(&p, 0, sizeof p);
                p.x_hi = hi(o.in); p.x_lo = lo(o.in); p.gate = h->se_gate; p.y_hi = hi(o.out); p.y_lo = lo(o.out);
                p.pitch = E.d.pitch;
                p.per_image = (long long)E.d.hw * E.d.hw * (E.d.pitch / 8);
                p.units = (long long)B * p.per_image;
                rc = launch_se_scale(h, p, o.conv, as_stream(stream));
                break;
            }
            case OP_AVGPOOLSILU: rc = mpx_global_avgpool_silu(h, hi(o.in), lo(o.in), hi(o.out), lo(o.out), B, o.hin * o.hin, o.c, stream); break;
            case OP_SHUFFLE: {
                const ShuffleOp& S = h->shuffles[o.conv];
                ShuffleParams p;
                std::memset(&p, 0, sizeof p);
                p.a_hi = hi(o.in); p.a_lo = lo(o.in); p.b_hi = hi(o.res) + S.b_offset; p.b_lo = lo(o.res) + S.b_offset;
                p.y_hi = hi(o.out); p.y_lo = lo(o.out);
                p.npix = (long long)B * S.side * S.side;
                p.a_pitch = S.a_pitch; p.b_pitch = S.b_pitch; p.bf = S.bf; p.hp = S.hp;
                rc = launch_shuffle(h, p, o.conv, as_stream(stream));
                break;
            }
            case OP_CATNORM: {
                const NormLayer& nl = h->norms[o.conv];
                CatNormParams p;
                std::memset(&p, 0, sizeof p);
                p.f_hi = hi(o.in); p.f_lo = lo(o.in); p.r_hi = hi(o.res); p.r_lo = lo(o.res); p.y_hi = hi(o.out); p.y_lo = lo(o.out);
                p.scale = nl.scale; p.shift = nl.shift;
                p.npix = (long long)B * o.hin * o.hin;
                p.f_stride = o.g; p.c_total = o.ctot; p.c_old = o.c - o.g; p.c_begin = 0; p.c_end = o.c;
                rc = launch_catnorm(h, p, o.conv, as_stream(stream));
                break;
            }
        }
        if (rc) return rc;
    }
    return 0;
}

int mpx_stem_conv_maxpool(mpx_engine* h, void* out_hi, void* out_lo, int B, void* stream) {
    if (!h) return MPX_E_ARG;
    if (!out_hi || !out_lo || B <= 0) return fail(h, MPX_E_ARG, "stem + max pool: null pointer or empty batch");
    if (B > h->max_batch) return fail(h, MPX_E_STATE, "stem + max pool: B=%d exceeds max_batch=%d", B, h->max_batch);
    MPX_SET_DEVICE(h);
    return launch_stem_pool(h, (half_t*)out_hi, (half_t*)out_lo, B, as_stream(stream));
}

int mpx_set_fusion(mpx_engine* h, int mask) {
    if (!h) return MPX_E_ARG;
    h->fuse_pool = (mask & 1) != 0;
    h->fuse_ds = (mask & 1) != 0;
    h->fuse_bt = (mask & 2) != 0;
    return 0;
}

int mpx_bottleneck_tail(mpx_engine* h, int i, const void* t1_hi, const void* t1_lo, const void* x_hi, const void* x_lo,
                        void* out_hi, void* out_lo, void* next_hi, void* next_lo, int B, void* stream) {
    if (!h) return MPX_E_ARG;
    if (B <= 0 || (t1_hi == nullptr) != (t1_lo == nullptr) || !x_hi || !x_lo || !out_hi || !out_lo || !next_hi || !next_lo)
        return fail(h, MPX_E_ARG, "bottleneck_tail: null planes or empty batch");
    int ti = -1;
    for (size_t k = 0; k < h->tails.size(); ++k)
        if (h->tails[k].c2 == i) ti = (int)k;
    if (ti < 0) return fail(h, MPX_E_ARG, "bottleneck_tail: layer %d is not the conv2 of a block whose tail runs as one launch", i);
    {
        const TailBlock& tb = h->tails[ti];
        const size_t px = (size_t)B * h->convs[tb.c2].d.hin * h->convs[tb.c2].d.hin * sizeof(half_t);
        const size_t c_x = tb.ds >= 0 ? BT_MID : BT_OUT, c_next = (size_t)h->convs[tb.next1].d.cout;
        struct Range { const char* lo; size_t n; const char* what; };
        const Range r[8] = {{(const char*)t1_hi, px * BT_MID, "t1_hi"}, {(const char*)t1_lo, px * BT_MID, "t1_lo"},
                            {(const char*)x_hi, px * c_x, "x_hi"}, {(const char*)x_lo, px * c_x, "x_lo"},
                            {(const char*)out_hi, px * BT_OUT, "out_hi"}, {(const char*)out_lo, px * BT_OUT, "out_lo"},
                            {(const char*)next_hi, px * c_next, "next_hi"}, {(const char*)next_lo, px * c_next, "next_lo"}};
        for (int a = 0; a < 8; ++a)
            for (int b = a + 1; b < 8; ++b)
                if (r[a].lo && r[b].lo && r[a].lo < r[b].lo + r[b].n && r[b].lo < r[a].lo + r[a].n)
                    return fail(h, MPX_E_ARG, "bottleneck_tail: planes %s and %s overlap (all plane pairs must be distinct buffers)", r[a].what, r[b].what);
    }
    MPX_SET_DEVICE(h);
    return launch_btail(h, ti, (const half_t*)t1_hi, (const half_t*)t1_lo, (const half_t*)x_hi, (const half_t*)x_lo, (half_t*)out_hi,
                        (half_t*)out_lo, (half_t*)next_hi, (half_t*)next_lo, B, as_stream(stream));
}

int mpx_num_bottleneck_tails(const mpx_engine* h) { return h ? (int)h->tails.size() : MPX_E_ARG; }

int mpx_bottleneck_tail_info(const mpx_engine* h, int k, int* conv2, int* conv3, int* downsample, int* next_conv1) {
    if (!h || k < 0 || k >= (int)h->tails.size()) return MPX_E_ARG;
    if (conv2) *conv2 = h->tails[k].c2;
    if (conv3) *conv3 = h->tails[k].c3;
    if (downsample) *downsample = h->tails[k].ds;
    if (next_conv1) *next_conv1 = h->tails[k].next1;
    return 0;
}

int mpx_conv_dual_bn_act(mpx_engine* h, int i, const void* in_hi, const void* in_lo, const void* x_hi, const void* x_lo,
                         void* out_hi, void* out_lo, int B, void* stream) {
    if (!h) return MPX_E_ARG;
    if (i < 0 || i >= (int)h->convs.size() || B <= 0) return fail(h, MPX_E_ARG, "conv_dual_bn_act: bad layer index or batch");
    if (!h->convs[i].fuse_main) return fail(h, MPX_E_ARG, "conv_dual_bn_act: layer %d (%s) is not the last conv of a block with a downsample branch", i, h->convs[i].d.name);
    if (!in_hi || !in_lo || !x_hi || !x_lo || !out_hi || !out_lo) return fail(h, MPX_E_ARG, "conv_dual_bn_act: null planes");
    MPX_SET_DEVICE(h);
    return launch_conv_fused(h, i, (const half_t*)in_hi, (const half_t*)in_lo, (const half_t*)x_hi, (const half_t*)x_lo,
                             (half_t*)out_hi, (half_t*)out_lo, B, as_stream(stream));
}

int mpx_heatmap_accumulate(mpx_engine* h, const int32_t* seg, const uint8_t* onoff, const int32_t* pred,
                           const int32_t* label, int M, int S, float* heat, void* stream) {
    if (!h) return MPX_E_ARG;
    if (!seg || !onoff || !pred || !label || !heat || M <= 0 || S <= 0 || S > 4096)
        return fail(h, MPX_E_ARG, "heatmap_accumulate: null pointer, empty M/S or S > 4096");
    MPX_SET_DEVICE(h);
    hipStream_t st = as_stream(stream);
    hipLaunchKernelGGL(heatmap_segment_count_kernel, dim3((S + 255) / 256), dim3(256), 0, st, onoff, pred, label, M, S,
                       h->seg_scratch);
    MPX_HIP(h, hipGetLastError());
    const int npix = h->img * h->img;
    hipLaunchKernelGGL(heatmap_gather_kernel, dim3((npix + 255) / 256), dim3(256), 0, st, seg, h->seg_scratch, S, npix, heat);
    MPX_HIP(h, hipGetLastError());
    return 0;
}

int mpx_input_planes(const mpx_engine* h, void** hi, void** lo) {
    if (!h || !hi || !lo) return MPX_E_ARG;
    *hi = h->in_hi;
    *lo = h->in_lo;
    return 0;
}

int mpx_mark_input_staged(mpx_engine* h, int slot0, int M) {
    if (!h) return MPX_E_ARG;
    if (slot0 < 0 || M <= 0 || (long long)slot0 + M > h->max_batch)
        return fail(h, MPX_E_ARG, "mark_input_staged: slots [%d, %d) outside [0, max_batch=%d)", slot0, slot0 + M, h->max_batch);
    if (h->in_forward) return fail(h, MPX_E_STATE, "mark_input_staged: called during mpx_forward");
    std::fill(h->slot_src.begin() + slot0, h->slot_src.begin() + slot0 + M, (uint8_t)1);
    return 0;
}

int mpx_stem_planes(const mpx_engine* h, void** hi, void** lo) {
    if (!h || !hi || !lo) return MPX_E_ARG;
    *hi = h->stem_hi;
    *lo = h->stem_lo;
    return 0;
}

int mpx_profile_enable(mpx_engine* h, int on) {
    if (!h) return MPX_E_ARG;
    if (on && h->prof_pool.empty()) {
        MPX_SET_DEVICE(h);
        h->prof_pool.resize(kProfilePairs);
        for (ProfRec& r : h->prof_pool) {
            MPX_HIP(h, hipEventCreate(&r.t0));
            MPX_HIP(h, hipEventCreate(&r.t1));
        }
    }
    h->prof_on = on != 0;
    return 0;
}

int mpx_profile_collect(mpx_engine* h, double ms_by_kind[4], long long launches_by_kind[4], double* per_conv_ms) {
    return mpx_profile_collect_ex(h, ms_by_kind, launches_by_kind, per_conv_ms, nullptr, nullptr);
}

int mpx_profile_collect_ex(mpx_engine* h, double ms_by_kind[4], long long launches_by_kind[4], double* per_conv_ms,
                           double* per_norm_ms, double* avgpool2_ms) {
    return mpx_profile_collect_dw(h, ms_by_kind, launches_by_kind, per_conv_ms, per_norm_ms, avgpool2_ms, nullptr);
}

int mpx_profile_collect_dw(mpx_engine* h, double ms_by_kind[4], long long launches_by_kind[4], double* per_conv_ms,
                           double* per_norm_ms, double* avgpool2_ms, double* per_dw_ms) {
    return mpx_profile_collect_pool(h, ms_by_kind, launches_by_kind, per_conv_ms, per_norm_ms, avgpool2_ms, per_dw_ms, nullptr);
}

int mpx_profile_collect_pool(mpx_engine* h, double ms_by_kind[4], long long launches_by_kind[4], double* per_conv_ms,
                             double* per_norm_ms, double* avgpool2_ms, double* per_dw_ms, double* per_clip_pool_ms) {
    return mpx_profile_collect_shuffle(h, ms_by_kind, launches_by_kind, per_conv_ms, per_norm_ms, avgpool2_ms, per_dw_ms, per_clip_pool_ms, nullptr);
}

int mpx_profile_collect_shuffle(mpx_engine* h, double ms_by_kind[4], long long launches_by_kind[4], double* per_conv_ms,
                                double* per_norm_ms, double* avgpool2_ms, double* per_dw_ms, double* per_clip_pool_ms, double* per_shuffle_ms) {
    return mpx_profile_collect_se(h, ms_by_kind, launches_by_kind, per_conv_ms, per_norm_ms, avgpool2_ms, per_dw_ms, per_clip_pool_ms, per_shuffle_ms,
                                  nullptr, nullptr);
}

int mpx_profile_collect_se(mpx_engine* h, double ms_by_kind[4], long long launches_by_kind[4], double* per_conv_ms, double* per_norm_ms,
                           double* avgpool2_ms, double* per_dw_ms, double* per_clip_pool_ms, double* per_shuffle_ms, double* per_se_gate_ms,
                           double* per_se_scale_ms) {
    if (!h || !ms_by_kind || !launches_by_kind) return MPX_E_ARG;
    if (h->prof_used == 0) return 0;
    MPX_SET_DEVICE(h);
    MPX_HIP(h, hipEventSynchronize(h->prof_pool[h->prof_used - 1].t1));
    for (int i = 0; i < h->prof_used; ++i) {
        ProfRec& r = h->prof_pool[i];
        float ms = 0.f;
        MPX_HIP(h, hipEventElapsedTime(&ms, r.t0, r.t1));
        ms_by_kind[r.kind] += ms;
        launches_by_kind[r.kind] += 1;
        if (per_conv_ms && r.kind == OP_CONV && r.conv >= 0) per_conv_ms[r.conv] += ms;
        if (per_norm_ms && r.kind == 2 && r.sub >= 0 && r.sub < (int)h->norms.size()) per_norm_ms[r.sub] += ms;
        if (avgpool2_ms && r.kind == 2 && r.sub == -2) *avgpool2_ms += ms;
        if (per_dw_ms && r.kind == 2 && r.sub <= kProfSubDw && kProfSubDw - r.sub < (int)h->dws.size()) per_dw_ms[kProfSubDw - r.sub] += ms;
        if (per_clip_pool_ms && r.kind == 2 && r.sub <= kProfSubPool3c && kProfSubPool3c - r.sub < (int)h->pools3c.size())
            per_clip_pool_ms[kProfSubPool3c - r.sub] += ms;
        if (per_shuffle_ms && r.kind == 2 && r.sub <= kProfSubShuffle && kProfSubShuffle - r.sub < (int)h->shuffles.size())
            per_shuffle_ms[kProfSubShuffle - r.sub] += ms;
        if (per_se_gate_ms && r.kind == 2 && r.sub <= kProfSubSeGate && kProfSubSeGate - r.sub < (int)h->ses.size())
            per_se_gate_ms[kProfSubSeGate - r.sub] += ms;
        if (per_se_scale_ms && r.kind == 2 && r.sub <= kProfSubSeScale && kProfSubSeScale - r.sub < (int)h->ses.size())
            per_se_scale_ms[kProfSubSeScale - r.sub] += ms;
    }
    h->prof_used = 0;
    return 0;
}

#ifdef MPX_DIAG
int mpx_debug_set_stamps(mpx_engine* h, void* dev_buf) {
    if (!h) return MPX_E_ARG;
    h->stamps = (unsigned long long*)dev_buf;
    return 0;
}
#endif

double mpx_flops_per_forward(const mpx_engine* h) {
    if (!h) return 0.0;
    double macs = 0.0;
    for (const ConvLayer& L : h->convs)
        macs += (double)L.d.hout * L.d.hout * L.d.cout * L.d.cin * L.d.ksize * L.d.ksize;
    for (const DwLayer& D : h->dws) {
        const int ho = (D.d.hin - 1) / D.d.stride + 1;
        macs += (double)ho * ho * D.d.channels * D.ksize * D.ksize;
    }
    for (const SeLayer& E : h->ses) macs += 2.0 * E.d.channels * E.d.q;
    return 2.0 * macs;
}

}
```

network_interpretation_imagenet_amd/csrc/mpx_btail.h:

```cpp
#pragma once
#include "mpx_conv.h"
#include <type_traits>

namespace mpx {

struct BtParams {
    const half_t* t_hi;
    const half_t* t_lo;
    const half_t* w0_hi;
    const half_t* w0_lo;
    const float* sc0;
    const float* sh0;
    const half_t* w2_hi;
    const half_t* w2_lo;
    const float* sc2;
    const float* sh2;
    const half_t* w3_hi;
    const half_t* w3_lo;
    const float* sc3;
    const float* sh3;
    const half_t* r_hi;
    const half_t* r_lo;
    half_t* y_hi;
    half_t* y_lo;
// ... 482 lines not shown
                        const float r = fmaxf(v[j], 0.f);
                        const half_t hi = (half_t)r;
                        t2h[s][b][half * 4 + j] = hi;
                        t2l[s][b][half * 4 + j] = (half_t)__builtin_fmaf((float)hi, -one, r);
                    }
                }
            }

#pragma unroll
        for (int a = 0; a < 4 * H1; ++a)
#pragma unroll
            for (int b = 0; b < 2; ++b) acc1[a][b] = (f4){0.f, 0.f, 0.f, 0.f};

        auto chunk = [&](auto c_tag) {
            constexpr int c = decltype(c_tag)::value;
            constexpr int J0 = JC + c * SC;
            f4 acc3[4][2];
#pragma unroll
            for (int a = 0; a < 4; ++a)
#pragma unroll
                for (int b = 0; b < 2; ++b) acc3[a][b] = (f4){0.f, 0.f, 0.f, 0.f};
            step(std::integral_constant<int, J0>{}, acc3, t2h[0], t2l[0]);
            step(std::integral_constant<int, J0 + 1>{}, acc3, t2h[1], t2l[1]);
            if constexpr (DUAL) {
                step(std::integral_constant<int, J0 + 2>{}, acc3, x0h[0], x0l[0]);
                step(std::integral_constant<int, J0 + 3>{}, acc3, x0h[1], x0l[1]);
            }
            __builtin_amdgcn_sched_barrier(0);
            BT_PHASE(bt_ph[2]);
#pragma unroll
            for (int a = 0; a < 4; ++a) {
                const f4 sc = *(const f4*)(vec + V_SC3 + c * 64 + a * 16 + 4 * lg);
                const f4 sh = *(const f4*)(vec + V_SH3 + c * 64 + a * 16 + 4 * lg);
#pragma unroll
                for (int b = 0; b < 2; ++b) *(f4*)(stg + (b * 16 + lp) * 256 + (((a * 4 + lg) ^ lp) << 4)) = acc3[a][b] * sc + sh;
            }
#pragma unroll
            for (int b = 0; b < 2; ++b) {
                f4 v0[2], v1[2];
#pragma unroll
                for (int k = 0; k < 2; ++k) {
                    const int slot = (2 * b + k) * 8 + (lane >> 3);
                    v0[k] = *(const f4*)(stg + slot * 256 + (((2 * uq) ^ (slot & 15)) << 4));
                    v1[k] = *(const f4*)(stg + slot * 256 + (((2 * uq + 1) ^ (slot & 15)) << 4));
                }
#pragma unroll
                for (int k = 0; k < 2; ++k) {
                    const int u = 2 * b + k;
                    const int slot = u * 8 + (lane >> 3);
                    float v[8] = {v0[k][0], v0[k][1], v0[k][2], v0[k][3], v1[k][0], v1[k][1], v1[k][2], v1[k][3]};
                    if (!DUAL) {
                        const h8 a8 = __builtin_bit_cast(h8, idh[u]);
                        const h8 c8 = __builtin_bit_cast(h8, idl[u]);
#pragma unroll
                        for (int j = 0; j < 8; ++j) v[j] = __builtin_fmaf((float)c8[j], one, __builtin_fmaf((float)a8[j], one, v[j]));
                    }
                    h8 oh, ol;
                    bt_relu_split8(v, one, oh, ol);
                    const int voff = (u_pix[u] * (BT_OUT * 2) + uq * 16) | (u_pix[u] & (int)OOB) | ((BT_ABL & 4) ? (int)OOB : 0);
                    __builtin_amdgcn_raw_buffer_store_b128(__builtin_bit_cast(u4, oh), yh, voff, c * 128, BT_AUX_STORE);
                    __builtin_amdgcn_raw_buffer_store_b128(__builtin_bit_cast(u4, ol), yl, voff, c * 128, BT_AUX_STORE);
                    char* const d = stg + (b * 4 + (uq >> 2) * 2) * 1024 + (slot & 15) * 64 + (((uq & 3) ^ (((slot >> 3) & 1) << 1)) << 4);
                    *(h8*)d = oh;
                    *(h8*)(d + 1024) = ol;
                }
            }
            if (C::late_a(J0 + S3 - 1)) {
#pragma unroll
                for (int i = 0; i < 8; ++i) read_a1((sbase + J0 + S3) & 3, fa[(J0 + S3) & 1], i);
            }
#pragma unroll
            for (int b = 0; b < 2; ++b) {
                cb[0].hi[b] = *(const h8*)(stg + (b * 4 + 0) * 1024 + sb_off);
                cb[0].lo[b] = *(const h8*)(stg + (b * 4 + 1) * 1024 + sb_off);
            }
            __builtin_amdgcn_sched_barrier(0);
            BT_PHASE(bt_ph[3]);
            step(std::integral_constant<int, J0 + S3>{}, &acc1[0], cb[0].hi, cb[0].lo);
            if constexpr (H1 == 1) {
                step(std::integral_constant<int, J0 + S3 + 1>{}, &acc1[0], cb[1].hi, cb[1].lo);
            } else {
                step(std::integral_constant<int, J0 + S3 + 1>{}, &acc1[4], cb[0].hi, cb[0].lo);
                step(std::integral_constant<int, J0 + S3 + 2>{}, &acc1[0], cb[1].hi, cb[1].lo);
                step(std::integral_constant<int, J0 + S3 + 3>{}, &acc1[4], cb[1].hi, cb[1].lo);
            }
            BT_PHASE(bt_ph[4]);
        };
        chunk(std::integral_constant<int, 0>{});
        chunk(std::integral_constant<int, 1>{});
        chunk(std::integral_constant<int, 2>{});
        chunk(std::integral_constant<int, 3>{});

        __builtin_amdgcn_sched_barrier(0);
        h8 zoh[4], zol[4];
#pragma unroll
        for (int hb = 0; hb < H1; ++hb) {
#pragma unroll
            for (int a = 0; a < 4; ++a) {
                const f4 sc = *(const f4*)(vec + V_SC1 + hb * 64 + a * 16 + 4 * lg);
                const f4 sh = *(const f4*)(vec + V_SH1 + hb * 64 + a * 16 + 4 * lg);
#pragma unroll
                for (int b = 0; b < 2; ++b) *(f4*)(stg + (b * 16 + lp) * 256 + (((a * 4 + lg) ^ lp) << 4)) = acc1[hb * 4 + a][b] * sc + sh;
            }
#pragma unroll
            for (int u = 0; u < 4; ++u) {
                const int slot = u * 8 + (lane >> 3);
                const f4 w0 = *(const f4*)(stg + slot * 256 + (((2 * uq) ^ (slot & 15)) << 4));
                const f4 w1 = *(const f4*)(stg + slot * 256 + (((2 * uq + 1) ^ (slot & 15)) << 4));
                const float v[8] = {w0[0], w0[1], w0[2], w0[3], w1[0], w1[1], w1[2], w1[3]};
                bt_relu_split8(v, one, zoh[u], zol[u]);
                if (hb + 1 < H1) {
                    const int voff = (u_pix[u] * (C1 * 2) + uq * 16) | (u_pix[u] & (int)OOB) | ((BT_ABL & 4) ? (int)OOB : 0);
                    __builtin_amdgcn_raw_buffer_store_b128(__builtin_bit_cast(u4, zoh[u]), zh, voff, hb * 128, BT_AUX_STORE);
                    __builtin_amdgcn_raw_buffer_store_b128(__builtin_bit_cast(u4, zol[u]), zl, voff, hb * 128, BT_AUX_STORE);
                }
            }
        }
        __builtin_amdgcn_sched_barrier(0);
        asm volatile("s_waitcnt lgkmcnt(0)" ::: "memory");
        BT_SUB(0);
        __builtin_amdgcn_s_barrier();
        __builtin_amdgcn_sched_barrier(0);
        BT_SUB(2);
        if (it + 1 < my_tiles) issue_patch(it + 1);
        __builtin_amdgcn_sched_barrier(0);
        BT_SUB(4);
#pragma unroll
        for (int u = 0; u < 4; ++u) {
            const int voff = (u_pix[u] * (C1 * 2) + uq * 16) | (u_pix[u] & (int)OOB) | ((BT_ABL & 4) ? (int)OOB : 0);
            __builtin_amdgcn_raw_buffer_store_b128(__builtin_bit_cast(u4, zoh[u]), zh, voff, (H1 - 1) * 128, BT_AUX_STORE);
            __builtin_amdgcn_raw_buffer_store_b128(__builtin_bit_cast(u4, zol[u]), zl, voff, (H1 - 1) * 128, BT_AUX_STORE);
        }
        __builtin_amdgcn_sched_barrier(0);
        BT_SUB(3);
        sbase = (sbase + NSTEP) & 3;
        BT_PHASE(bt_ph[5]);
    }
    wait_vmcnt<0>();
#ifdef MPX_DIAG
    if (p.stamps && tid == 0) {
        unsigned long long* o_ = p.stamps + (size_t)blockIdx.x * 8;
#pragma unroll
        for (int i = 0; i < 6; ++i) o_[i] = bt_ph[i];
        o_[6] = __builtin_amdgcn_s_memtime() - bt_t0;
        o_[7] = (unsigned long long)my_tiles;
        unsigned long long* q_ = p.stamps + (size_t)(gridDim.x + blockIdx.x) * 8;
#pragma unroll
        for (int i = 0; i < 5; ++i) q_[i] = bt_sub[i];
    }
#endif
#endif
}

typedef BtCfg<false, 64> BtResC64;
typedef BtCfg<false, 128> BtResC128;
typedef BtCfg<true, 64> BtDualC64;
typedef BtCfg<true, 64, true> BtHeadC64;

static_assert(BtResC64::NSTEP == 34 && BtResC128::NSTEP == 42 && BtDualC64::NSTEP == 42, "steps per tile");
static_assert(BtResC64::wait_top(14) == 4 && BtResC64::wait_top(16) == 12 && BtResC64::wait_top(18) == 12 && BtResC64::wait_top(19) == 4,
              "conv2 -> chunk 0");
static_assert(BtResC64::wait_top(20) == 12 && BtResC64::wait_top(21) == 20 && BtResC64::wait_top(22) == 20 && BtResC64::wait_top(23) == 12,
              "chunk pattern: conv1' steps behind the stores, the next chunk's conv3 steps behind the identity loads");
static_assert(BtResC64::wait_top(0) == 20 && BtDualC64::wait_top(4) == 12 && BtDualC64::wait_top(6) == 4, "tile start; block-input loads of the DUAL tail in step 2");

}
```

network_interpretation_imagenet_amd/engine.py:

```python
import ctypes as C

import numpy as np
import torch

from . import _lib
from ._lib import MpxError, IMG, NUM_CLASSES

MEAN = (0.485, 0.456, 0.406)
STD = (0.229, 0.224, 0.225)
BN_EPS = 1e-5
GOOGLENET_BN_EPS = 1e-3

ARCH_IDS = {"resnet18": 18, "resnet34": 34, "resnet50": 50, "resnet101": 101, "resnet152": 152,
            "mnist_net": 1, "cifar_resnet20": 2020, "cifar_resnet56": 2056, "cifar_resnet110": 2110}
ARCH_IDS.update({"vgg%d%s" % (d, bn): (3100 if bn else 3000) + d for d in (11, 13, 16, 19) for bn in ("", "_bn")})
ARCH_IDS["alexnet"] = 4000
ARCH_IDS.update({"densenet%d" % d: 5000 + d for d in (121, 169, 201)})
ARCH_IDS["mobilenet_v2"] = 6002
ARCH_IDS["squeezenet1_1"] = 7011
ARCH_IDS["googlenet"] = 8000
ARCH_IDS.update({"shufflenet_v2_x0_5": 9005, "shufflenet_v2_x1_0": 9010, "shufflenet_v2_x1_5": 9015, "shufflenet_v2_x2_0": 9020})
ARCH_IDS["efficientnet_b0"] = 10000


# ... 411 lines not shown
                logits[s0:s0 + b] = out[2].cpu().numpy()
        return (onoff, score, pred, logits) if return_logits else (onoff, score, pred)

    def score_packed(self, images, segs, onoffs, label_rows, score_out, pred_out, stem=None):
        n = len(images)
        shared = isinstance(segs, torch.Tensor)
        if len(onoffs) != n or (not shared and len(segs) != n):
            raise ValueError("images, segs and onoffs must have one entry per image")
        total = sum(int(o.shape[0]) for o in onoffs)
        for name, t, dt in (("label_rows", label_rows, torch.int32), ("score_out", score_out, torch.float32), ("pred_out", pred_out, torch.int32)):
            if t.dtype != dt or t.device != self.device or t.numel() != total or not t.is_contiguous():
                raise ValueError("%s must be contiguous %s[%d] on %s" % (name, dt, total, self.device))
        label_rows, score_out, pred_out = label_rows.view(-1), score_out.view(-1), pred_out.view(-1)
        done = 0
        used = 0
        used_kind = None
        if stem is not None:
            self._staging(stem, 0)

        def flush():
            nonlocal done, used
            self.forward(used, label_rows[done:done + used], score_out=score_out[done:done + used], pred_out=pred_out[done:done + used])
            done += used
            used = 0

        for i in range(n):
            m, r = int(onoffs[i].shape[0]), 0
            if not m:
                continue
            seg = segs if shared else segs[i]
            kind = self.stem_for_rows(m) if stem is None else stem
            if used and kind != used_kind:
                flush()
            used_kind = kind
            if kind == "table":
                self.build_stem_table(images[i], seg, int(onoffs[i].shape[1]))
            while r < m:
                take = min(m - r, self.max_batch - used)
                if kind == "table":
                    self.apply_stem_table(onoffs[i][r:r + take], used)
                else:
                    self.stage_masks(images[i], seg, onoffs[i][r:r + take], used)
                used += take
                r += take
                if used == self.max_batch:
                    flush()
        if used:
            flush()

    def score_images(self, images, segments, onoffs, labels, stem=None):
        if self.small:
            raise ValueError("%s scores with score_masks_removed (the small networks' mask convention)" % self.arch)
        n = len(images)
        if not (len(segments) == len(onoffs) == len(labels) == n):
            raise ValueError("images, segments, onoffs and labels must have the same length")
        self._staging(stem, 0)
        img_d, seg_d, onoff_d, lab, sizes = [], [], [], [], []
        for i in range(n):
            seg_rank, s = rank_segments(segments[i])
            o = np.ascontiguousarray(onoffs[i])
            if o.dtype != np.uint8 or o.ndim != 2 or o.shape[1] != s:
                raise ValueError("onoffs[%d] must be uint8[M,%d] (S = number of distinct segment labels), got %s%s" % (i, s, o.dtype, o.shape))
            if not 0 <= int(labels[i]) < NUM_CLASSES:
                raise ValueError("label %r outside [0,1000)" % (labels[i],))
            sizes.append(o.shape[0])
            if o.shape[0] == 0:
                continue
            img_d.append(self._image_to_device(images[i]))
            seg_d.append(torch.from_numpy(seg_rank).to(self.device))
            onoff_d.append(torch.from_numpy(o).to(self.device))
            lab.append(np.full(o.shape[0], int(labels[i]), dtype=np.int32))
        total = int(sum(sizes))
        if total == 0:
            return [(np.empty(0, np.float32), np.empty(0, np.int32)) for _ in range(n)]
        order = list(range(len(img_d)))
        if stem is None:
            order.sort(key=lambda k: self.stem_for_rows(int(onoff_d[k].shape[0])) != "table")
        label_rows = torch.from_numpy(np.concatenate([lab[k] for k in order])).to(self.device)
        score = torch.empty(total, dtype=torch.float32, device=self.device)
        pred = torch.empty(total, dtype=torch.int32, device=self.device)
        self.score_packed([img_d[k] for k in order], [seg_d[k] for k in order], [onoff_d[k] for k in order], label_rows, score, pred, stem=stem)
        score, pred = score.cpu().numpy(), pred.cpu().numpy()
        packed, at = {}, 0
        for k in order:
            m = int(onoff_d[k].shape[0])
            packed[k] = (score[at:at + m].copy(), pred[at:at + m].copy())
            at += m
        out, k = [], 0
        for m in sizes:
            if m == 0:
                out.append((np.empty(0, np.float32), np.empty(0, np.int32)))
            else:
                out.append(packed[k])
                k += 1
        return out

    def predict(self, image):
        seg = np.zeros((IMG, IMG), dtype=np.int32)
        _o, _s, pred, logits = self.score_masks(image, seg, np.ones((1, 1), dtype=np.uint8), 0, return_logits=True)
        z = logits[0].astype(np.float64)
        p = np.exp(z - z.max())
        return int(pred[0]), (p / p.sum()).astype(np.float32)

    def heatmap_accumulate(self, seg, onoff, pred, labels, heat):
        m, s = onoff.shape
        for name, t, dt in (("seg", seg, torch.int32), ("onoff", onoff, torch.uint8), ("pred", pred, torch.int32),
                            ("labels", labels, torch.int32), ("heat", heat, torch.float32)):
            if t.device != self.device or t.dtype != dt or not t.is_contiguous():
                raise ValueError("%s must be a contiguous %s tensor on %s" % (name, dt, self.device))
        if tuple(seg.shape) != (IMG, IMG) or tuple(heat.shape) != (IMG, IMG) or pred.numel() != m or labels.numel() != m:
            raise ValueError("shapes: seg/heat [224,224], pred/labels [M], onoff [M,S]")
        _lib.check(self._h, self._lib.mpx_heatmap_accumulate(self._h, _ptr(seg), _ptr(onoff), _ptr(pred), _ptr(labels),
                                                             int(m), int(s), _ptr(heat), self._stream()),
                   "mpx_heatmap_accumulate")
        return heat

    def heatmap_device(self, image, seg_rank, onoff, label, buf, stem=None):
        if buf.dtype != torch.float32 or buf.device != self.device or buf.numel() != IMG * IMG + 1 or not buf.is_contiguous():
            raise ValueError("buf must be a contiguous float32[%d] tensor on %s" % (IMG * IMG + 1, self.device))
        seg_rank, s = rank_segments(seg_rank)
        onoff = np.ascontiguousarray(onoff)
        if onoff.dtype != np.uint8 or onoff.ndim != 2 or onoff.shape[1] != s:
            raise ValueError("onoff must be uint8[M,%d] (S = number of distinct segment labels), got %s%s" % (s, onoff.dtype, onoff.shape))
        if not 0 <= int(label) < NUM_CLASSES:
            raise ValueError("label %r outside [0,1000)" % (label,))
        m = int(onoff.shape[0])
        self._staging(stem, m)
        score = torch.empty(m, dtype=torch.float32, device=self.device)
        pred = torch.empty(m, dtype=torch.int32, device=self.device)
        if m == 0:
            return score, pred
        seg_d = torch.from_numpy(seg_rank).to(self.device)
        onoff_d = torch.from_numpy(onoff).to(self.device)
        labels = torch.full((m,), int(label), dtype=torch.int32, device=self.device)
        self.score_packed([self._image_to_device(image)], seg_d, [onoff_d], labels, score, pred, stem=stem)
        self.heatmap_accumulate(seg_d, onoff_d, pred, labels, buf[:IMG * IMG].view(IMG, IMG))
        buf[IMG * IMG] += (pred == labels).sum()
        return score, pred

    def heatmap(self, seg_rank, onoff, pred, label):
        m = int(np.asarray(onoff).shape[0])
        heat = torch.zeros(IMG, IMG, dtype=torch.float32, device=self.device)
        if m:
            t = lambda a, dt: torch.from_numpy(np.ascontiguousarray(a, dtype=dt)).to(self.device)
            self.heatmap_accumulate(t(seg_rank, np.int32), t(onoff, np.uint8), t(pred, np.int32),
                                    torch.full((m,), int(label), dtype=torch.int32, device=self.device), heat)
        return heat.cpu().numpy().astype(np.float64)

    def set_conv_tile(self, layer, tile):
        i = layer if isinstance(layer, int) else [d.name.decode() for d in self.layers].index(layer)
        _lib.check(self._h, self._lib.mpx_set_conv_tile(self._h, int(i), int(tile)), "mpx_set_conv_tile")

    def set_fusion(self, on=True):
        mask = (3 if on else 0) if isinstance(on, bool) else int(on)
        _lib.check(self._h, self._lib.mpx_set_fusion(self._h, mask), "mpx_set_fusion")

    def bottleneck_tails(self):
        out = []
        for k in range(self._lib.mpx_num_bottleneck_tails(self._h)):
            v = [C.c_int() for _ in range(4)]
            _lib.check(self._h, self._lib.mpx_bottleneck_tail_info(self._h, k, *[C.byref(x) for x in v]), "mpx_bottleneck_tail_info")
            out.append(tuple(int(x.value) for x in v))
        return out

    def conv_tile(self, layer):
        i = layer if isinstance(layer, int) else [d.name.decode() for d in self.layers].index(layer)
        return int(self._lib.mpx_get_conv_tile(self._h, int(i)))

    def profile(self, on=True):
        _lib.check(self._h, self._lib.mpx_profile_enable(self._h, 1 if on else 0), "mpx_profile_enable")

    def collect_profile(self):
        ms = (C.c_double * 4)()
        n = (C.c_longlong * 4)()
        per = (C.c_double * len(self.layers))()
        per_norm = (C.c_double * max(1, len(self.norms)))()
        avg2 = (C.c_double * 1)()
        per_dw = (C.c_double * max(1, len(self.dwconvs)))()
        n_cp = int(self._lib.mpx_num_clip_pools(self._h))
        per_cp = (C.c_double * max(1, n_cp))()
        n_sh = int(self._lib.mpx_num_shuffles(self._h))
        per_sh = (C.c_double * max(1, n_sh))()
        per_sg = (C.c_double * max(1, len(self.ses)))()
        per_ss = (C.c_double * max(1, len(self.ses)))()
        _lib.check(self._h, self._lib.mpx_profile_collect_se(self._h, ms, n, per, per_norm, avg2, per_dw, per_cp, per_sh, per_sg, per_ss), "mpx_profile_collect_se")
        kinds = ("conv", "mask_apply_normalize", "pool", "head")
        return {"ms": dict(zip(kinds, list(ms))), "launches": dict(zip(kinds, list(n))),
                "per_conv_ms": list(per), "per_norm_ms": list(per_norm)[:len(self.norms)], "avgpool2_ms": float(avg2[0]),
                "per_dw_ms": list(per_dw)[:len(self.dwconvs)], "per_clip_pool_ms": list(per_cp)[:n_cp], "per_shuffle_ms": list(per_sh)[:n_sh],
                "per_se_gate_ms": list(per_sg)[:len(self.ses)], "per_se_scale_ms": list(per_ss)[:len(self.ses)]}
```

Baseline: 23250 masked-forward-passes/s.

## Fuse conv3 plus residual with next block's conv1 in layer2 bottlenecks

Adds a pointwise-tail kernel that computes a bottleneck's 1x1 conv3 (128->512) with BN, residual add and ReLU, stores the block output, and feeds that output tile from LDS straight into the next block's 1x1 conv1 (512->128) with BN+ReLU. This removes one launch per block and the re-read of the 512-channel output for the next conv1. The op planner gets new op lists (with and without the existing bottleneck-tail fusion), a fusion-mask bit, and a fallback to two separate convs when tiles are non-default. The cost is a large hand-scheduled kernel with high LDS use (72KB) at two blocks per CU, and a risk of losing the per-layer tuned conv kernels.

```diff
diff --git a/include/mpx.h b/include/mpx.h
--- a/include/mpx.h
+++ b/include/mpx.h
@@ -133,6 +133,11 @@
                         void* out_hi, void* out_lo, void* next_hi, void* next_lo, int B, void* stream);
 int mpx_num_bottleneck_tails(const mpx_engine* h);
 int mpx_bottleneck_tail_info(const mpx_engine* h, int k, int* conv2, int* conv3, int* downsample, int* next_conv1);
+
+int mpx_pointwise_tail(mpx_engine* h, int i, const void* t2_hi, const void* t2_lo, const void* x_hi, const void* x_lo,
+                       void* out_hi, void* out_lo, void* next_hi, void* next_lo, int B, void* stream);
+int mpx_num_pointwise_tails(const mpx_engine* h);
+int mpx_pointwise_tail_info(const mpx_engine* h, int k, int* conv3, int* next_conv1);
 
 int mpx_maxpool3x3s2(mpx_engine* h, const void* in_hi, const void* in_lo, void* out_hi,
                      void* out_lo, int B, int hin, int c, void* stream);
diff --git a/network_interpretation_imagenet_amd/_lib.py b/network_interpretation_imagenet_amd/_lib.py
--- a/network_interpretation_imagenet_amd/_lib.py
+++ b/network_interpretation_imagenet_amd/_lib.py
@@ -67,6 +67,9 @@
     "mpx_bottleneck_tail": (_i, [_vp, _i, _vp, _vp, _vp, _vp, _vp, _vp, _vp, _vp, _i, _vp]),
     "mpx_num_bottleneck_tails": (_i, [_vp]),
     "mpx_bottleneck_tail_info": (_i, [_vp, _i, C.POINTER(_i), C.POINTER(_i), C.POINTER(_i), C.POINTER(_i)]),
+    "mpx_pointwise_tail": (_i, [_vp, _i, _vp, _vp, _vp, _vp, _vp, _vp, _vp, _vp, _i, _vp]),
+    "mpx_num_pointwise_tails": (_i, [_vp]),
+    "mpx_pointwise_tail_info": (_i, [_vp, _i, C.POINTER(_i), C.POINTER(_i)]),
     "mpx_stem_conv_maxpool": (_i, [_vp, _vp, _vp, _i, _vp]),
     "mpx_maxpool3x3s2": (_i, [_vp, _vp, _vp, _vp, _vp, _i, _i, _i, _vp]),
     "mpx_maxpool2x2s2": (_i, [_vp, _vp, _vp, _vp, _vp, _i, _i, _i, _vp]),
diff --git a/network_interpretation_imagenet_amd/csrc/mpx_api.hip b/network_interpretation_imagenet_amd/csrc/mpx_api.hip
--- a/network_interpretation_imagenet_amd/csrc/mpx_api.hip
+++ b/network_interpretation_imagenet_amd/csrc/mpx_api.hip
@@ -43,7 +43,7 @@
 
 enum OpKind { OP_CONV = 0, OP_MAXPOOL = 1, OP_AVGPOOL = 2, OP_HEAD = 3, OP_AVGPAD = 4, OP_BTAIL = 5, OP_MAXPOOL2 = 6, OP_MAXPOOL3P0 = 7,
               OP_CATNORM = 8, OP_AVGPOOL2 = 9, OP_DWCONV = 10, OP_AVGPOOL6 = 11, OP_AVGLOGITS = 12, OP_MAXPOOL3C = 13, OP_SHUFFLE = 14,
-              OP_SEGATE = 15, OP_SESCALE = 16, OP_AVGPOOLSILU = 17 };
+              OP_SEGATE = 15, OP_SESCALE = 16, OP_AVGPOOLSILU = 17, OP_PTAIL = 18 };
 enum Buf { BUF_INPUT = -1, BUF_POOL = -2, BUF_NONE = -3, BUF_STEM = -4 };
 
 struct ConvLayer {
@@ -102,6 +102,10 @@
     bool ready = false;
 };
 
+struct PointTail {
+    int c3 = -1, next1 = -1;
+};
+
 struct DwLayer {
     mpx_dwconv_desc d;
     bool linear = false;
@@ -178,6 +182,11 @@
     std::vector<TailBlock> tails;
     int ops_bt_x = 0;
     bool fuse_bt = true;
+    std::vector<Op> ops_pt;
+    std::vector<Op> ops_pt0;
+    std::vector<PointTail> ptails;
+    int ops_pt_x = 0, ops_pt0_x = 0;
+    bool fuse_pt = true;
     char* arena = nullptr;
     size_t arena_bytes = 0;
     char* tab_arena = nullptr;
@@ -390,10 +399,17 @@
             return n1.cin == BT_OUT && n1.ksize == 1 && n1.stride == 1 && n1.hin == 56 && (n1.cout == 64 || n1.cout == 128) &&
                    !(blocks[k].ds >= 0 && n1.cout != 64);
         };
+        auto ptail_ok = [&](size_t k) {
+            if (k + 1 >= blocks.size() || blocks[k].ds >= 0 || tail_ok(k)) return false;
+            const mpx_conv_desc& d3 = h->convs[blocks[k].c3].d;
+            const mpx_conv_desc& n1 = h->convs[blocks[k + 1].c1].d;
+            return d3.cin == BtPw128::MID && d3.cout == BtPw128::OUT && d3.ksize == 1 && d3.stride == 1 && d3.residual == 1 &&
+                   n1.cin == BtPw128::OUT && n1.cout == BtPw128::C1 && n1.ksize == 1 && n1.stride == 1 && n1.hin == d3.hin;
+        };
         bool any = false;
         for (size_t k = 0; k < blocks.size(); ++k) any |= tail_ok(k);
-        if (any) {
-            std::vector<Op>& out = h->ops_bt;
+        auto plan = [&](std::vector<Op>& out, bool bt, bool pt, bool rec_bt, bool rec_pt) {
+            size_t n_bt = 0, n_pt = 0;
             out.push_back(h->ops[0]);
             out.push_back(h->ops[1]);
             int Xb = BUF_STEM, T1c = -100;
@@ -403,20 +419,22 @@
 #ifdef BT_NO_HEAD
                 const bool whole = false;
 #else
-                const bool whole = tail_ok(k) && R.ds >= 0 && T1 < 0;
+                const bool whole = bt && tail_ok(k) && R.ds >= 0 && T1 < 0;
 #endif
                 if (T1 < 0 && !whole) {
                     T1 = pick({Xb});
                     out.push_back(Op{OP_CONV, R.c1, Xb, T1, BUF_NONE, 0, 0, BUF_NONE});
                 }
                 T1c = -100;
-                if (tail_ok(k)) {
-                    TailBlock tb;
-                    tb.c1 = R.c1; tb.c2 = R.c2; tb.c3 = R.c3; tb.ds = R.ds; tb.next1 = blocks[k + 1].c1;
-                    h->tails.push_back(tb);
+                if (bt && tail_ok(k)) {
+                    if (rec_bt) {
+                        TailBlock tb;
+                        tb.c1 = R.c1; tb.c2 = R.c2; tb.c3 = R.c3; tb.ds = R.ds; tb.next1 = blocks[k + 1].c1;
+                        h->tails.push_back(tb);
+                    }
                     if (whole) T1 = BUF_NONE;
                     const int O = pick({Xb, T1}), Z = pick({Xb, T1, O});
-                    Op o{OP_BTAIL, (int)h->tails.size() - 1, T1, O, Xb, 0, 0, BUF_NONE};
+                    Op o{OP_BTAIL, (int)n_bt++, T1, O, Xb, 0, 0, BUF_NONE};
                     o.z = Z;
                     out.push_back(o);
                     Xb = O;
@@ -425,6 +443,16 @@
                 }
                 const int T2 = pick({Xb, T1});
                 out.push_back(Op{OP_CONV, R.c2, T1, T2, BUF_NONE, 0, 0, BUF_NONE});
+                if (pt && ptail_ok(k)) {
+                    if (rec_pt) h->ptails.push_back(PointTail{R.c3, blocks[k + 1].c1});
+                    const int O = pick({Xb, T2}), Z = pick({Xb, T2, O});
+                    Op o{OP_PTAIL, (int)n_pt++, T2, O, Xb, 0, 0, BUF_NONE};
+                    o.z = Z;
+                    out.push_back(o);
+                    Xb = O;
+                    T1c = Z;
+                    continue;
+                }
                 int res = Xb;
                 if (R.ds >= 0) {
                     const int T3 = pick({Xb, T1, T2});
@@ -434,7 +462,14 @@
                 out.push_back(Op{OP_CONV, R.c3, T2, T1, res, 0, 0, R.ds >= 0 ? Xb : BUF_NONE});
                 Xb = T1;
             }
-            h->ops_bt_x = Xb;
+            return Xb;
+        };
+        bool any_pt = false;
+        for (size_t k = 0; k < blocks.size(); ++k) any_pt |= ptail_ok(k);
+        if (any) h->ops_bt_x = plan(h->ops_bt, true, false, true, false);
+        if (any_pt) {
+            h->ops_pt0_x = plan(h->ops_pt0, false, true, false, true);
+            if (any) h->ops_pt_x = plan(h->ops_pt, true, true, false, false);
         }
     }
     h->feat = cin;
@@ -443,10 +478,11 @@
     h->convs[c].is_fc = true;
     add_op(OP_CONV, c, BUF_POOL, BUF_NONE, BUF_NONE, 0, 0);
     add_op(OP_HEAD, -1, BUF_NONE, BUF_NONE, BUF_NONE, 0, 0);
-    if (!h->ops_bt.empty()) {
-        h->ops_bt.push_back(Op{OP_AVGPOOL, -1, h->ops_bt_x, BUF_POOL, BUF_NONE, hcur, cin, BUF_NONE});
-        h->ops_bt.push_back(h->ops[h->ops.size() - 2]);
-        h->ops_bt.push_back(h->ops[h->ops.size() - 1]);
+    for (auto lx : {std::make_pair(&h->ops_bt, h->ops_bt_x), std::make_pair(&h->ops_pt, h->ops_pt_x), std::make_pair(&h->ops_pt0, h->ops_pt0_x)}) {
+        if (lx.first->empty()) continue;
+        lx.first->push_back(Op{OP_AVGPOOL, -1, lx.second, BUF_POOL, BUF_NONE, hcur, cin, BUF_NONE});
+        lx.first->push_back(h->ops[h->ops.size() - 2]);
+        lx.first->push_back(h->ops[h->ops.size() - 1]);
     }
     return 0;
 }
@@ -1454,6 +1490,7 @@
     {(const void*)btail_f16x3_kernel<BtResC128>, BtResC128::LDS},
     {(const void*)btail_f16x3_kernel<BtDualC64>, BtDualC64::LDS},
     {(const void*)btail_f16x3_kernel<BtHeadC64>, BtHeadC64::LDS},
+    {(const void*)btail_f16x3_kernel<BtPw128>, BtPw128::LDS},
     {(const void*)conv3x3p_f16x3_kernel<PatchTile0>, kLdsLimit},
     {(const void*)conv3x3p_f16x3_kernel<PatchTile1>, kLdsLimit},
     {(const void*)conv3x3p_f16x3_kernel<PatchTile2>, kLdsLimit},
@@ -1694,6 +1731,40 @@
     else hipLaunchKernelGGL(btail_f16x3_kernel<BtResC64>, dim3(grid), dim3(256), BtResC64::LDS, st, p);
     MPX_HIP(h, hipGetLastError());
     return 0;
+}
+
+int launch_ptail(mpx_engine* h, int ti, const half_t* t_hi, const half_t* t_lo, const half_t* x_hi, const half_t* x_lo,
+                 half_t* y_hi, half_t* y_lo, half_t* z_hi, half_t* z_lo, int B, hipStream_t st) {
+    const PointTail& pt = h->ptails[ti];
+    const ConvLayer& L3 = h->convs[pt.c3];
+    const ConvLayer& N1 = h->convs[pt.next1];
+    if (!L3.loaded || !N1.loaded) return fail(h, MPX_E_STATE, "pointwise tail %s: weights missing", L3.d.name);
+    if (L3.d.k_packed != BtPw128::MID || N1.d.k_packed != BtPw128::OUT) return fail(h, MPX_E_INTERNAL, "pointwise tail %s: packed K %d / %d", L3.d.name, L3.d.k_packed, N1.d.k_packed);
+    BtParams p;
+    std::memset(&p, 0, sizeof p);
+    p.t_hi = t_hi; p.t_lo = t_lo;
+    p.w3_hi = L3.w_hi; p.w3_lo = L3.w_lo; p.sc3 = L3.scale; p.sh3 = L3.shift;
+    p.r_hi = x_hi; p.r_lo = x_lo; p.y_hi = y_hi; p.y_lo = y_lo;
+    p.w1_hi = N1.w_hi; p.w1_lo = N1.w_lo; p.sc1 = N1.scale; p.sh1 = N1.shift;
+    p.z_hi = z_hi; p.z_lo = z_lo;
+    p.B = B; p.H = L3.d.hin; p.W = L3.d.hin;
+    const long long M = (long long)B * p.H * p.W;
+    const long long n_tiles = (M + BtPw128::TP - 1) / BtPw128::TP;
+    if (n_tiles <= 0 || M > 0x7fffffffLL) return fail(h, MPX_E_ARG, "pointwise tail: batch out of range");
+    p.n_tiles = (int)n_tiles;
+    const long long resident = 2LL * h->num_cus;
+    const unsigned grid = (unsigned)std::min<long long>(resident, n_tiles);
+    ProfScope ps(h, st, OP_CONV, pt.c3);
+    hipLaunchKernelGGL(btail_f16x3_kernel<BtPw128>, dim3(grid), dim3(256), BtPw128::LDS, st, p);
+    MPX_HIP(h, hipGetLastError());
+    return 0;
+}
+
+bool ptail_in_use(const mpx_engine* h, int k) {
+    const PointTail& pt = h->ptails[k];
+    for (int li : {pt.c3, pt.next1})
+        if (!h->convs[li].loaded || h->convs[li].tile != default_tile(h->convs[li].d)) return false;
+    return true;
 }
 
 int build_fused(mpx_engine* h, int main) {
@@ -2845,13 +2916,22 @@
     for (const TailBlock& tb : h->tails)
         for (int li : {tb.c1, tb.c2, tb.c3, tb.next1})
             use_bt = use_bt && h->convs[li].tile == default_tile(h->convs[li].d);
-    const std::vector<Op>& ops = use_bt ? h->ops_bt : h->ops;
+    const bool use_pt = h->fuse_pt && h->fuse_ds && !h->ptails.empty();
+    const std::vector<Op>& ops = use_pt ? (use_bt ? h->ops_pt : h->ops_pt0) : (use_bt ? h->ops_bt : h->ops);
     for (size_t oi = 0; oi < ops.size(); ++oi) {
         const Op& o = ops[oi];
         if (stem_done && ((o.kind == OP_CONV && o.conv == 0) || (o.kind == OP_MAXPOOL && o.out == BUF_STEM))) continue;
         switch (o.kind) {
             case OP_BTAIL:
                 rc = launch_btail(h, o.conv, hi(o.in), lo(o.in), hi(o.res), lo(o.res), hi(o.out), lo(o.out), hi(o.z), lo(o.z), B, as_stream(stream));
+                break;
+            case OP_PTAIL:
+                if (ptail_in_use(h, o.conv)) {
+                    rc = launch_ptail(h, o.conv, hi(o.in), lo(o.in), hi(o.res), lo(o.res), hi(o.out), lo(o.out), hi(o.z), lo(o.z), B, as_stream(stream));
+                    break;
+                }
+                rc = mpx_conv_bn_act(h, h->ptails[o.conv].c3, hi(o.in), lo(o.in), hi(o.res), lo(o.res), hi(o.out), lo(o.out), nullptr, B, stream);
+                if (!rc) rc = mpx_conv_bn_act(h, h->ptails[o.conv].next1, hi(o.out), lo(o.out), nullptr, nullptr, hi(o.z), lo(o.z), nullptr, B, stream);
                 break;
             case OP_CONV:
                 if (h->fuse_pool && o.conv == 0 && oi + 1 < ops.size() && ops[oi + 1].kind == OP_MAXPOOL && stem_pool_eligible(h) &&
@@ -2977,6 +3057,7 @@
     h->fuse_pool = (mask & 1) != 0;
     h->fuse_ds = (mask & 1) != 0;
     h->fuse_bt = (mask & 2) != 0;
+    h->fuse_pt = (mask & 4) != 0;
     return 0;
 }
 
@@ -3019,6 +3100,42 @@
     return 0;
 }
 
+int mpx_pointwise_tail(mpx_engine* h, int i, const void* t2_hi, const void* t2_lo, const void* x_hi, const void* x_lo,
+                       void* out_hi, void* out_lo, void* next_hi, void* next_lo, int B, void* stream) {
+    if (!h) return MPX_E_ARG;
+    if (B <= 0 || !t2_hi || !t2_lo || !x_hi || !x_lo || !out_hi || !out_lo || !next_hi || !next_lo)
+        return fail(h, MPX_E_ARG, "pointwise_tail: null planes or empty batch");
+    int ti = -1;
+    for (size_t k = 0; k < h->ptails.size(); ++k)
+        if (h->ptails[k].c3 == i) ti = (int)k;
+    if (ti < 0) return fail(h, MPX_E_ARG, "pointwise_tail: layer %d is not the conv3 of a block whose pointwise tail runs as one launch", i);
+    {
+        const PointTail& pt = h->ptails[ti];
+        const size_t px = (size_t)B * h->convs[pt.c3].d.hin * h->convs[pt.c3].d.hin * sizeof(half_t);
+        struct Range { const char* lo; size_t n; const char* what; };
+        const Range r[8] = {{(const char*)t2_hi, px * BtPw128::MID, "t2_hi"}, {(const char*)t2_lo, px * BtPw128::MID, "t2_lo"},
+                            {(const char*)x_hi, px * BtPw128::OUT, "x_hi"}, {(const char*)x_lo, px * BtPw128::OUT, "x_lo"},
+                            {(const char*)out_hi, px * BtPw128::OUT, "out_hi"}, {(const char*)out_lo, px * BtPw128::OUT, "out_lo"},
+                            {(const char*)next_hi, px * BtPw128::C1, "next_hi"}, {(const char*)next_lo, px * BtPw128::C1, "next_lo"}};
+        for (int a = 0; a < 8; ++a)
+            for (int b = a + 1; b < 8; ++b)
+                if (r[a].lo < r[b].lo + r[b].n && r[b].lo < r[a].lo + r[a].n)
+                    return fail(h, MPX_E_ARG, "pointwise_tail: planes %s and %s overlap (all plane pairs must be distinct buffers)", r[a].what, r[b].what);
+    }
+    MPX_SET_DEVICE(h);
+    return launch_ptail(h, ti, (const half_t*)t2_hi, (const half_t*)t2_lo, (const half_t*)x_hi, (const half_t*)x_lo, (half_t*)out_hi,
+                        (half_t*)out_lo, (half_t*)next_hi, (half_t*)next_lo, B, as_stream(stream));
+}
+
+int mpx_num_pointwise_tails(const mpx_engine* h) { return h ? (int)h->ptails.size() : MPX_E_ARG; }
+
+int mpx_pointwise_tail_info(const mpx_engine* h, int k, int* conv3, int* next_conv1) {
+    if (!h || k < 0 || k >= (int)h->ptails.size()) return MPX_E_ARG;
+    if (conv3) *conv3 = h->ptails[k].c3;
+    if (next_conv1) *next_conv1 = h->ptails[k].next1;
+    return 0;
+}
+
 int mpx_conv_dual_bn_act(mpx_engine* h, int i, const void* in_hi, const void* in_lo, const void* x_hi, const void* x_lo,
                          void* out_hi, void* out_lo, int B, void* stream) {
     if (!h) return MPX_E_ARG;
diff --git a/network_interpretation_imagenet_amd/csrc/mpx_btail.h b/network_interpretation_imagenet_amd/csrc/mpx_btail.h
--- a/network_interpretation_imagenet_amd/csrc/mpx_btail.h
+++ b/network_interpretation_imagenet_amd/csrc/mpx_btail.h
@@ -658,16 +658,338 @@
 #endif
 }
 
+template <int C1_>
+struct BtPwCfg {
+    static constexpr int C1 = C1_;
+    static constexpr int MID = 128, OUT = 512;
+    static constexpr int TP = 128;
+    static constexpr int NCH = OUT / 64;
+    static constexpr int S3 = MID / 32;
+    static constexpr int H1 = C1 / 64;
+    static constexpr int S1 = 2 * H1;
+    static constexpr int SC = S3 + S1;
+    static constexpr int NSTEP = NCH * SC;
+    static constexpr int JT = NSTEP - S1;
+    static constexpr int NVEC = 2 * (OUT + C1);
+    static constexpr int OFF_STG = 8192;
+    static constexpr int OFF_RING = OFF_STG + 4 * 8192;
+    static constexpr int LDS = OFF_RING + BT_NRING * BT_STAGE;
+    static_assert(NVEC * 4 <= OFF_STG, "vectors overflow their LDS area");
+    static_assert(C1 == 128, "conv1' has 128 output channels");
+    static_assert(NSTEP % BT_NRING == 0, "ring slot of a step = step % 4 in every tile (and the fragment parity with it)");
+
+    static constexpr int mod(int j) { return ((j % NSTEP) + NSTEP) % NSTEP; }
+    static constexpr int pre(int j) {
+        j = mod(j);
+        return (j % SC == 0 ? 8 : 0) + (j == JT ? 4 * S3 : 0);
+    }
+    static constexpr int post(int j) {
+        j = mod(j);
+        return (j % SC == S3 - 1 ? 8 : 0) + (j == NSTEP - 1 ? 8 * H1 : 0);
+    }
+    static constexpr int all(int j) { return 2 + pre(j) + post(j); }
+    static constexpr bool late_a(int j) { return mod(j) % SC < S3; }
+    static constexpr int wait_top(int j) { return pre(j - 3) + post(j - 3) + all(j - 2) + all(j - 1); }
+};
+
+template <class C>
+__device__ __forceinline__ void btail_pointwise_body(const BtParams& p) {
+#if defined(__HIP_DEVICE_COMPILE__)
+    extern __shared__ __attribute__((aligned(16))) char smem[];
+    typedef unsigned u4 __attribute__((ext_vector_type(4)));
+    constexpr int C1 = C::C1, MID = C::MID, OUT = C::OUT, TP = C::TP, NCH = C::NCH, S3 = C::S3, S1 = C::S1, SC = C::SC, H1 = C::H1, NSTEP = C::NSTEP;
+
+    const int tid = threadIdx.x;
+    const int lane = tid & 63;
+    const int wave = __builtin_amdgcn_readfirstlane(tid >> 6);
+    const int lp = lane & 15, lg = lane >> 4;
+    float one = 1.0f;
+    asm volatile("" : "+s"(one));
+
+    const long long M = (long long)p.B * p.H * p.W;
+    const int G = gridDim.x;
+    const int v0 = blockIdx.x;
+    if (v0 >= p.n_tiles) return;
+    const int my_tiles = (p.n_tiles - 1 - v0) / G + 1;
+
+    char* const ring = smem + C::OFF_RING;
+    char* const stg = smem + C::OFF_STG + wave * 8192;
+    float* const vec = (float*)smem;
+    constexpr int V_SC3 = 0, V_SH3 = OUT, V_SC1 = 2 * OUT, V_SH1 = 2 * OUT + C1;
+    for (int i = tid; i < C::NVEC; i += 256) {
+        float v;
+        if (i < V_SH3) v = p.sc3[i];
+        else if (i < V_SC1) v = p.sh3[i - V_SH3];
+        else if (i < V_SH1) v = p.sc1[i - V_SC1];
+        else v = p.sh1[i - V_SH1];
+        vec[i] = v;
+    }
+
+    const __amdgpu_buffer_rsrc_t w3h = __builtin_amdgcn_make_buffer_rsrc((void*)p.w3_hi, 0, OUT * MID * 2, 0x00020000);
+    const __amdgpu_buffer_rsrc_t w3l = __builtin_amdgcn_make_buffer_rsrc((void*)p.w3_lo, 0, OUT * MID * 2, 0x00020000);
+    const __amdgpu_buffer_rsrc_t w1h = __builtin_amdgcn_make_buffer_rsrc((void*)p.w1_hi, 0, C1 * OUT * 2, 0x00020000);
+    const __amdgpu_buffer_rsrc_t w1l = __builtin_amdgcn_make_buffer_rsrc((void*)p.w1_lo, 0, C1 * OUT * 2, 0x00020000);
+    const int w_lane = lane * 16;
+    auto issue_stage = [&](auto js_tag, int slot) {
+        constexpr int JS = decltype(js_tag)::value;
+        constexpr int cc = JS / SC, r = JS % SC;
+        char* const d = ring + slot * BT_STAGE + wave * 1024;
+        if (r < S3) {
+            const int soff = ((4 * cc + wave) * S3 + r) * 1024;
+            __builtin_amdgcn_raw_ptr_buffer_load_lds(w3h, MPX_LDS_PTR(d), 16, w_lane, soff, 0, 0);
+            __builtin_amdgcn_raw_ptr_buffer_load_lds(w3l, MPX_LDS_PTR(d + 4096), 16, w_lane, soff, 0, 0);
+        } else {
+            constexpr int r1 = r - S3, kk = r1 / H1, hb = r1 % H1;
+            const int soff = ((4 * hb + wave) * (OUT / 32) + 2 * cc + kk) * 1024;
+            __builtin_amdgcn_raw_ptr_buffer_load_lds(w1h, MPX_LDS_PTR(d), 16, w_lane, soff, 0, 0);
+            __builtin_amdgcn_raw_ptr_buffer_load_lds(w1l, MPX_LDS_PTR(d + 4096), 16, w_lane, soff, 0, 0);
+        }
+    };
+
+    const int a_off = lp * 64 + ((lg ^ (((lane >> 3) & 1) << 1)) << 4);
+    const int sb_off = lp * 64 + ((lg ^ (((lp >> 3) & 1) << 1)) << 4);
+    const int uq = lane & 7;
+    const int y_voff = (wave * 32 + (lane >> 3)) * (OUT * 2) + uq * 16;
+    const int z_voff = (wave * 32 + (lane >> 3)) * (C1 * 2) + uq * 16;
+    const int t_voff = (wave * 32 + lp) * (MID * 2) + lg * 16;
+    auto tile_rsrc = [&](const half_t* base, int t, int ch) {
+        const long long pix0 = (long long)t * TP;
+        const long long rem = M - pix0;
+        const int rows = rem < 0 ? 0 : (rem > TP ? TP : (int)rem);
+        return __builtin_amdgcn_make_buffer_rsrc((void*)(base + pix0 * ch), 0, rows * ch * 2, 0x00020000);
+    };
+
+    f4 acc1[4 * H1][2];
+    h8 t2h[S3][2], t2l[S3][2];
+    u4 idh[4], idl[4];
+    struct FragA { h8 hi[4], lo[4]; };
+    struct FragB { h8 hi[2], lo[2]; };
+    FragA fa[2];
+    FragB cb[2];
+
+    auto issue_t2 = [&](int t) {
+        const __amdgpu_buffer_rsrc_t th = tile_rsrc(p.t_hi, t, MID);
+        const __amdgpu_buffer_rsrc_t tl = tile_rsrc(p.t_lo, t, MID);
+#pragma unroll
+        for (int b = 0; b < 2; ++b)
+#pragma unroll
+            for (int kk = 0; kk < S3; ++kk) {
+                t2h[kk][b] = __builtin_bit_cast(h8, __builtin_amdgcn_raw_buffer_load_b128(th, t_voff + b * 16 * MID * 2, kk * 64, 0));
+                t2l[kk][b] = __builtin_bit_cast(h8, __builtin_amdgcn_raw_buffer_load_b128(tl, t_voff + b * 16 * MID * 2, kk * 64, 0));
+            }
+    };
+    auto read_a1 = [&](int slot, FragA& f, int i) {
+        const char* s = ring + slot * BT_STAGE + a_off + (i & 3) * 1024;
+        if (i < 4) f.hi[i] = *(const h8*)s;
+        else f.lo[i - 4] = *(const h8*)(s + 4096);
+    };
+
+    issue_stage(std::integral_constant<int, 0>{}, 0);
+    issue_stage(std::integral_constant<int, 1>{}, 1);
+    issue_stage(std::integral_constant<int, 2>{}, 2);
+    issue_stage(std::integral_constant<int, 3>{}, 3);
+    issue_t2(v0);
+    __builtin_amdgcn_sched_barrier(0);
+    wait_vmcnt<0>();
+    __builtin_amdgcn_s_barrier();
+    __builtin_amdgcn_sched_barrier(0);
+#pragma unroll
+    for (int i = 0; i < 8; ++i) read_a1(0, fa[0], i);
+
+    for (int it = 0; it < my_tiles; ++it) {
+        const int t = v0 + it * G;
+        const __amdgpu_buffer_rsrc_t rh_rs = tile_rsrc(p.r_hi, t, OUT);
+        const __amdgpu_buffer_rsrc_t rl_rs = tile_rsrc(p.r_lo, t, OUT);
+        const __amdgpu_buffer_rsrc_t yh = tile_rsrc(p.y_hi, t, OUT);
+        const __amdgpu_buffer_rsrc_t yl = tile_rsrc(p.y_lo, t, OUT);
+        const __amdgpu_buffer_rsrc_t zh = tile_rsrc(p.z_hi, t, C1);
+        const __amdgpu_buffer_rsrc_t zl = tile_rsrc(p.z_lo, t, C1);
+        __builtin_amdgcn_sched_barrier(0);
+
+        auto issue_identity = [&](int c) {
+#pragma unroll
+            for (int u = 0; u < 4; ++u) {
+                idh[u] = __builtin_amdgcn_raw_buffer_load_b128(rh_rs, y_voff + u * 8 * OUT * 2, c * 128, BT_AUX_LOAD);
+                idl[u] = __builtin_amdgcn_raw_buffer_load_b128(rl_rs, y_voff + u * 8 * OUT * 2, c * 128, BT_AUX_LOAD);
+            }
+        };
+        auto step = [&](auto j_tag, f4 (*acc)[2], const h8 (&bh)[2], const h8 (&bl)[2]) {
+            constexpr int J = decltype(j_tag)::value;
+            constexpr int r = J % SC;
+            const FragA& A = fa[J & 1];
+            FragA& An = fa[(J + 1) & 1];
+            __builtin_amdgcn_sched_barrier(0);
+            wait_vmcnt<C::wait_top(J)>();
+            __builtin_amdgcn_s_barrier();
+            __builtin_amdgcn_sched_barrier(0);
+#pragma unroll
+            for (int i = 0; i < 24; ++i) {
+                const int a = i / 6, q = i % 6, term = q >> 1, b = q & 1;
+                if (term == 0) acc[a][b] = __builtin_amdgcn_mfma_f32_16x16x32_f16(A.hi[a], bl[b], acc[a][b], 0, 0, 0);
+                else if (term == 1) acc[a][b] = __builtin_amdgcn_mfma_f32_16x16x32_f16(A.lo[a], bh[b], acc[a][b], 0, 0, 0);
+                else acc[a][b] = __builtin_amdgcn_mfma_f32_16x16x32_f16(A.hi[a], bh[b], acc[a][b], 0, 0, 0);
+                __builtin_amdgcn_sched_barrier(0);
+                if ((i & 1) == 0 && i < 16 && !C::late_a(J)) {
+                    read_a1((J + 1) & 3, An, i >> 1);
+                    __builtin_amdgcn_sched_barrier(0);
+                }
+                if ((i & 1) == 0 && i >= 16 && r == S3 + H1 - 1) {
+                    const int k = (i - 16) >> 1, fb = k & 1, plane = k >> 1;
+                    const h8 f = *(const h8*)(stg + (fb * 4 + 2 + plane) * 1024 + sb_off);
+                    if (plane == 0) cb[1].hi[fb] = f;
+                    else cb[1].lo[fb] = f;
+                    __builtin_amdgcn_sched_barrier(0);
+                }
+                if (i == 1) {
+                    issue_stage(std::integral_constant<int, (J + 4) % NSTEP>{}, J & 3);
+                    __builtin_amdgcn_sched_barrier(0);
+                }
+                if (i == 5 && r == 0) {
+                    issue_identity(J / SC);
+                    __builtin_amdgcn_sched_barrier(0);
+                }
+                if (i == 5 && J == C::JT) {
+                    issue_t2(t + G);
+                    __builtin_amdgcn_sched_barrier(0);
+                }
+            }
+            if (C::late_a(J) && r != S3 - 1) {
+#pragma unroll
+                for (int i = 0; i < 8; ++i) read_a1((J + 1) & 3, An, i);
+                __builtin_amdgcn_sched_barrier(0);
+            }
+        };
+
+#pragma unroll
+        for (int a = 0; a < 4 * H1; ++a)
+#pragma unroll
+            for (int b = 0; b < 2; ++b) acc1[a][b] = (f4){0.f, 0.f, 0.f, 0.f};
+
+        auto chunk = [&](auto c_tag) {
+            constexpr int c = decltype(c_tag)::value;
+            constexpr int J0 = c * SC;
+            f4 acc3[4][2];
+#pragma unroll
+            for (int a = 0; a < 4; ++a)
+#pragma unroll
+                for (int b = 0; b < 2; ++b) acc3[a][b] = (f4){0.f, 0.f, 0.f, 0.f};
+            step(std::integral_constant<int, J0>{}, acc3, t2h[0], t2l[0]);
+            step(std::integral_constant<int, J0 + 1>{}, acc3, t2h[1], t2l[1]);
+            step(std::integral_constant<int, J0 + 2>{}, acc3, t2h[2], t2l[2]);
+            step(std::integral_constant<int, J0 + 3>{}, acc3, t2h[3], t2l[3]);
+            __builtin_amdgcn_sched_barrier(0);
+            int ln = lane;
+            asm volatile("" : "+v"(ln));
+            const int lp = ln & 15, lg = ln >> 4, uq = ln & 7, l8 = ln >> 3;
+#pragma unroll
+            for (int a = 0; a < 4; ++a) {
+                const f4 sc = *(const f4*)(vec + V_SC3 + c * 64 + a * 16 + 4 * lg);
+                const f4 sh = *(const f4*)(vec + V_SH3 + c * 64 + a * 16 + 4 * lg);
+#pragma unroll
+                for (int b = 0; b < 2; ++b) *(f4*)(stg + (b * 16 + lp) * 256 + (((a * 4 + lg) ^ lp) << 4)) = acc3[a][b] * sc + sh;
+            }
+#pragma unroll
+            for (int b = 0; b < 2; ++b) {
+                f4 v0[2], v1[2];
+#pragma unroll
+                for (int k = 0; k < 2; ++k) {
+                    const int slot = (2 * b + k) * 8 + l8;
+                    v0[k] = *(const f4*)(stg + slot * 256 + (((2 * uq) ^ (slot & 15)) << 4));
+                    v1[k] = *(const f4*)(stg + slot * 256 + (((2 * uq + 1) ^ (slot & 15)) << 4));
+                }
+#pragma unroll
+                for (int k = 0; k < 2; ++k) {
+                    const int u = 2 * b + k;
+                    const int slot = u * 8 + l8;
+                    float v[8] = {v0[k][0], v0[k][1], v0[k][2], v0[k][3], v1[k][0], v1[k][1], v1[k][2], v1[k][3]};
+                    const h8 a8 = __builtin_bit_cast(h8, idh[u]);
+                    const h8 c8 = __builtin_bit_cast(h8, idl[u]);
+#pragma unroll
+                    for (int j = 0; j < 8; ++j) v[j] = __builtin_fmaf((float)c8[j], one, __builtin_fmaf((float)a8[j], one, v[j]));
+                    h8 oh, ol;
+                    bt_relu_split8(v, one, oh, ol);
+                    __builtin_amdgcn_raw_buffer_store_b128(__builtin_bit_cast(u4, oh), yh, y_voff + u * 8 * OUT * 2, c * 128, BT_AUX_STORE);
+                    __builtin_amdgcn_raw_buffer_store_b128(__builtin_bit_cast(u4, ol), yl, y_voff + u * 8 * OUT * 2, c * 128, BT_AUX_STORE);
+                    char* const d = stg + (b * 4 + (uq >> 2) * 2) * 1024 + (slot & 15) * 64 + (((uq & 3) ^ (((slot >> 3) & 1) << 1)) << 4);
+                    *(h8*)d = oh;
+                    *(h8*)(d + 1024) = ol;
+                }
+            }
+            __builtin_amdgcn_sched_barrier(0);
+#pragma unroll
+            for (int i = 0; i < 8; ++i) read_a1((J0 + S3) & 3, fa[(J0 + S3) & 1], i);
+#pragma unroll
+            for (int b = 0; b < 2; ++b) {
+                cb[0].hi[b] = *(const h8*)(stg + (b * 4 + 0) * 1024 + sb_off);
+                cb[0].lo[b] = *(const h8*)(stg + (b * 4 + 1) * 1024 + sb_off);
+            }
+            __builtin_amdgcn_sched_barrier(0);
+            step(std::integral_constant<int, J0 + S3>{}, &acc1[0], cb[0].hi, cb[0].lo);
+            step(std::integral_constant<int, J0 + S3 + 1>{}, &acc1[4], cb[0].hi, cb[0].lo);
+            step(std::integral_constant<int, J0 + S3 + 2>{}, &acc1[0], cb[1].hi, cb[1].lo);
+            step(std::integral_constant<int, J0 + S3 + 3>{}, &acc1[4], cb[1].hi, cb[1].lo);
+        };
+        chunk(std::integral_constant<int, 0>{});
+        chunk(std::integral_constant<int, 1>{});
+        chunk(std::integral_constant<int, 2>{});
+        chunk(std::integral_constant<int, 3>{});
+        chunk(std::integral_constant<int, 4>{});
+        chunk(std::integral_constant<int, 5>{});
+        chunk(std::integral_constant<int, 6>{});
+        chunk(std::integral_constant<int, 7>{});
+
+        __builtin_amdgcn_sched_barrier(0);
+        int ln = lane;
+        asm volatile("" : "+v"(ln));
+        const int lp = ln & 15, lg = ln >> 4, uq = ln & 7, l8 = ln >> 3;
+#pragma unroll
+        for (int hb = 0; hb < H1; ++hb) {
+#pragma unroll
+            for (int a = 0; a < 4; ++a) {
+                const f4 sc = *(const f4*)(vec + V_SC1 + hb * 64 + a * 16 + 4 * lg);
+                const f4 sh = *(const f4*)(vec + V_SH1 + hb * 64 + a * 16 + 4 * lg);
+#pragma unroll
+                for (int b = 0; b < 2; ++b) *(f4*)(stg + (b * 16 + lp) * 256 + (((a * 4 + lg) ^ lp) << 4)) = acc1[hb * 4 + a][b] * sc + sh;
+            }
+#pragma unroll
+            for (int u = 0; u < 4; ++u) {
+                const int slot = u * 8 + l8;
+                const f4 w0 = *(const f4*)(stg + slot * 256 + (((2 * uq) ^ (slot & 15)) << 4));
+                const f4 w1 = *(const f4*)(stg + slot * 256 + (((2 * uq + 1) ^ (slot & 15)) << 4));
+                const float v[8] = {w0[0], w0[1], w0[2], w0[3], w1[0], w1[1], w1[2], w1[3]};
+                h8 zoh, zol;
+                bt_relu_split8(v, one, zoh, zol);
+                __builtin_amdgcn_raw_buffer_store_b128(__builtin_bit_cast(u4, zoh), zh, z_voff + u * 8 * C1 * 2, hb * 128, BT_AUX_STORE);
+                __builtin_amdgcn_raw_buffer_store_b128(__builtin_bit_cast(u4, zol), zl, z_voff + u * 8 * C1 * 2, hb * 128, BT_AUX_STORE);
+            }
+        }
+        __builtin_amdgcn_sched_barrier(0);
+    }
+    wait_vmcnt<0>();
+#endif
+}
+
 typedef BtCfg<false, 64> BtResC64;
 typedef BtCfg<false, 128> BtResC128;
 typedef BtCfg<true, 64> BtDualC64;
 typedef BtCfg<true, 64, true> BtHeadC64;
+typedef BtPwCfg<128> BtPw128;
+
+template <>
+__global__ __launch_bounds__(256, 2) void btail_f16x3_kernel<BtPw128>(const BtParams p) {
+    btail_pointwise_body<BtPw128>(p);
+}
 
 static_assert(BtResC64::NSTEP == 34 && BtResC128::NSTEP == 42 && BtDualC64::NSTEP == 42, "steps per tile");
 static_assert(BtResC64::wait_top(14) == 4 && BtResC64::wait_top(16) == 12 && BtResC64::wait_top(18) == 12 && BtResC64::wait_top(19) == 4,
               "conv2 -> chunk 0");
 static_assert(BtResC64::wait_top(20) == 12 && BtResC64::wait_top(21) == 20 && BtResC64::wait_top(22) == 20 && BtResC64::wait_top(23) == 12,
               "chunk pattern: conv1' steps behind the stores, the next chunk's conv3 steps behind the identity loads");
+static_assert(BtPw128::NSTEP == 64 && BtPw128::LDS == 73728, "steps per tile, LDS of the pointwise form");
+static_assert(BtPw128::wait_top(3) == 12 && BtPw128::wait_top(4) == 12 && BtPw128::wait_top(6) == 12 && BtPw128::wait_top(7) == 4 && BtPw128::wait_top(8) == 4,
+              "chunk pattern of the pointwise form");
+static_assert(BtPw128::wait_top(63) == 20 && BtPw128::wait_top(0) == 20 && BtPw128::wait_top(1) == 28 && BtPw128::wait_top(2) == 28,
+              "tile boundary of the pointwise form");
 static_assert(BtResC64::wait_top(0) == 20 && BtDualC64::wait_top(4) == 12 && BtDualC64::wait_top(6) == 4, "tile start; block-input loads of the DUAL tail in step 2");
 
 }
diff --git a/network_interpretation_imagenet_amd/engine.py b/network_interpretation_imagenet_amd/engine.py
--- a/network_interpretation_imagenet_amd/engine.py
+++ b/network_interpretation_imagenet_amd/engine.py
@@ -587,7 +587,7 @@
         _lib.check(self._h, self._lib.mpx_set_conv_tile(self._h, int(i), int(tile)), "mpx_set_conv_tile")
 
     def set_fusion(self, on=True):
-        mask = (3 if on else 0) if isinstance(on, bool) else int(on)
+        mask = (7 if on else 0) if isinstance(on, bool) else int(on)
         _lib.check(self._h, self._lib.mpx_set_fusion(self._h, mask), "mpx_set_fusion")
 
     def bottleneck_tails(self):
@@ -595,6 +595,14 @@
         for k in range(self._lib.mpx_num_bottleneck_tails(self._h)):
             v = [C.c_int() for _ in range(4)]
             _lib.check(self._h, self._lib.mpx_bottleneck_tail_info(self._h, k, *[C.byref(x) for x in v]), "mpx_bottleneck_tail_info")
+            out.append(tuple(int(x.value) for x in v))
+        return out
+
+    def pointwise_tails(self):
+        out = []
+        for k in range(self._lib.mpx_num_pointwise_tails(self._h)):
+            v = [C.c_int() for _ in range(2)]
+            _lib.check(self._h, self._lib.mpx_pointwise_tail_info(self._h, k, *[C.byref(x) for x in v]), "mpx_pointwise_tail_info")
             out.append(tuple(int(x.value) for x in v))
         return out
 
```

Measured after the change: 23520 masked-forward-passes/s, median of 6. +1.2%, better.
